# AutomationLabs-sh/AutomationLabsModelPredictiveControl.jl

Measured on AMD Instinct MI355X. Metric: MPC steps/s (batch=4096, nx=12, nu=4, N=30), higher is better.
Workload: dtype f64; 1 GPU; configs[1]: hover-linearised quadrotor nx=12 nu=4 N=30, 4096 instances per GPU, shared model, x0 amplitude classes 0.3/1.0/3.0 interleaved, cold start every step; batch_per_gpu=4096, global_batch=4096, seed=0x5eed0002, setup_ramp_steps=300, admm_max_iter=6, check_every=6, polish=1, warm_state_kept=False, parallelism=instances sharded over 1 GPU(s), 16-instance tile per workgroup

## Files before the change

automationlabsmodelpredictivecontrol.jl_amd/csrc/almpc_api.hip:

```cpp
#include "almpc_kernels.hip.h"
#include "almpc_design.hip.h"
#include "almpc_polish_gen.hip.h"
#include "almpc_fnn.hip.h"
#include "almpc_instance.hip.h"
#include "almpc_sqp.hip.h"
#include "almpc_comm.hip.h"
#include "almpc_riccati.hip.h"
#include "almpc_sdual.hip.h"
#include "almpc_host_math.h"
#include "almpc_switches.h"
#include "../../include/almpc.h"

#ifndef ALMPC_UNITY
#define ALMPC_KERNEL_INSTANCE(...) extern template __global__ __VA_ARGS__;
#include "instances/sdual_a.inc"
#include "instances/sdual_b.inc"
#include "instances/sdual_c.inc"
#include "instances/polish_gen.inc"
#include "instances/step.inc"
#include "instances/instance.inc"
#include "instances/design_a.inc"
#include "instances/design_b.inc"
#undef ALMPC_KERNEL_INSTANCE
#endif

#include <algorithm>
#include <chrono>
#include <cstdio>
#include <cstdlib>
#include <cmath>
#include <cstring>
#include <limits>
#include <string>
#include <thread>
#include <type_traits>
#include <vector>

using namespace almpc;

struct almpc_handle {
    int n = 0, m = 0, N = 0, batch = 0, nz = 0, nzs = 0, nrb = 0, ks = 0, ksf = 0, device = 0;
    uint32_t flags = 0;
    hipStream_t stream = nullptr;
    std::string err;
    bool designed = false;
    double rho = 0.1, sigma = 1e-6;
    std::vector<double> H, F, P, d;
    double *dMinvFrag = nullptr, *dVFrag = nullptr, *dHFrag = nullptr, *dFFrag = nullptr, *dG = nullptr;
    double *dD = nullptr, *dUmin = nullptr, *dUmax = nullptr, *dA = nullptr, *dB = nullptr;
    double *dXref = nullptr, *dUref = nullptr, *dFS = nullptr, *dV0S = nullptr, *dRho = nullptr;
    size_t ref_cap[3] = {0, 0, 0};
    double *wQ = nullptr, *wR = nullptr, *wS = nullptr;
    int rho_mode = 0;
    double* dRollM = nullptr;
    int roll_s = 0, roll_nb = 0;
    long xref_stride = 0, uref_stride = 0, fS_stride = 0;
    std::vector<double> hS;
    int useS = 0;
    double *dX0 = nullptr, *dXs = nullptr, *dZs = nullptr, *dYs = nullptr, *dV0 = nullptr, *dW = nullptr;
    double *dX = nullptr, *dEx = nullptr, *dU = nullptr, *dEu = nullptr;
    int32_t *dStatus = nullptr, *dIters = nullptr, *dPiters = nullptr, *dPerm = nullptr;
    uint32_t* dYflags = nullptr;
    bool state_valid = true;
    int num_cus = 256;
    Switches sw;
    int fuse_step = 1;
    double* dSglobal = nullptr;
    int32_t* dStartRows = nullptr;
    int terminal_eq = 0, has_box = 0, mc = 0, R = 0, Rs = 0, np_pairs = 0;
    double *dGhat = nullptr, *dGnorm = nullptr, *dXmin = nullptr, *dXmax = nullptr;
    int *dRowTraj = nullptr, *dRowEq = nullptr, *dRowXidx = nullptr, *dRowState = nullptr;
    double* dOvfSinv = nullptr;
    double* dVsPlain = nullptr;
    double* dPlain = nullptr;
    double* dS0Basis = nullptr;
    bool s0_basis_ok = false;
    int32_t* dOverflow = nullptr;
    int* dRowMap = nullptr;
    double *dGhatE = nullptr, *dWinvE = nullptr;
    int eq_proj = 0;
    bool ghat_inst = false;
    std::vector<double> boxmin, boxmax;
    double *lA = nullptr, *lB = nullptr, *lC = nullptr, *lE = nullptr;
    bool batched = false;
    bool ltv = false;
    double* bQ = nullptr;
    double *bA = nullptr, *bB = nullptr, *bMinv = nullptr, *bG = nullptr, *bHs = nullptr, *bFs = nullptr, *bVs = nullptr,
           *bD = nullptr, *bRho = nullptr, *bH = nullptr, *bF = nullptr;
    double *bPhi = nullptr, *bGk = nullptr, *bGam = nullptr, *bW = nullptr, *bWP = nullptr, *bP = nullptr;
    int* bFlag = nullptr;
    bool batched_alloc = false;
    bool minv_packed = false;
    struct Sqp {
        bool ready = false, started = false;
        int H = 0, L = 0, act = 0, net = 0, useR = 0, useS = 0;
        long sP = 0;
        double *W_in = nullptr, *W_h = nullptr, *b_h = nullptr, *W_out = nullptr;
        double *A = nullptr, *B = nullptr, *c = nullptr, *fval = nullptr, *ebar = nullptr, *qadd = nullptr;
        double *xref = nullptr, *uref = nullptr, *Q = nullptr, *R = nullptr, *S = nullptr;
        int* bad = nullptr;
        double* mer = nullptr;
        double *xback = nullptr, *uback = nullptr, *dxback = nullptr, *vback = nullptr;
        double mu = 0.0;
        int step_rule = 0;
        long since_start = 0;
        int structured_qp = 0;
        unsigned long long* stats = nullptr;
        int stats_cap = 0;
        int* sv = nullptr;
        double* kkt = nullptr;
        int* live_pin = nullptr;
        int hessian = 0;
        double *lam = nullptr, *Wlag = nullptr;
        int row_mult = 0;
        double* smu = nullptr;
    } sqp;
    struct Relin {
        bool ready = false;
        int H = 0, L = 0, act = 0, net = 0, useR = 0, useS = 0;
        double *W_in = nullptr, *W_h = nullptr, *b_h = nullptr, *W_out = nullptr;
        double *ulin = nullptr;
        double *Q = nullptr, *R = nullptr, *S = nullptr;
        double *gS = nullptr;
        bool have_prev = false;
        double *u0 = nullptr, *xnext = nullptr;
        double *Ascr = nullptr, *Bscr = nullptr;
        float ms_jac = 0, ms_design = 0, ms_step = 0;
        hipEvent_t ev[4] = {nullptr, nullptr, nullptr, nullptr};
    } relin;
    bool structured = false;
    struct Redo {
// ... 52 lines not shown
        hipStream_t s_in = nullptr;
        double* dX0dev[IO_DEPTH] = {nullptr, nullptr};
        hipEvent_t ev_in[IO_DEPTH] = {nullptr, nullptr};
        double* hX0[IO_DEPTH] = {nullptr, nullptr};
        double* dX0[IO_DEPTH] = {nullptr, nullptr};
        hipEvent_t ev_used[IO_DEPTH] = {nullptr, nullptr};
        bool used_pending[IO_DEPTH] = {false, false};
        int x0_slot = -1;
        double* dX0_own = nullptr;
        long x0_count = 0;
        double *hX[IO_DEPTH] = {nullptr, nullptr}, *hEx[IO_DEPTH] = {nullptr, nullptr}, *hU[IO_DEPTH] = {nullptr, nullptr},
               *hEu[IO_DEPTH] = {nullptr, nullptr}, *hU0[IO_DEPTH] = {nullptr, nullptr};
        int32_t* hInts[IO_DEPTH] = {nullptr, nullptr};
        double* dU0[IO_DEPTH] = {nullptr, nullptr};
        int32_t* dInts[IO_DEPTH] = {nullptr, nullptr};
        hipEvent_t ev_packed[IO_DEPTH] = {nullptr, nullptr};
        hipEvent_t ev_done[IO_DEPTH] = {nullptr, nullptr};
        hipEvent_t ev_big = nullptr;
        uint32_t want[IO_DEPTH] = {0, 0};
        long ticket[IO_DEPTH] = {-1, -1};
        long next_ticket = 0;
        bool big_copy_pending = false;
        int big_copy_slot = 0;
    } io;
    std::vector<hipEvent_t> ev;
    std::vector<char> ev_two;
    size_t ev_used = 0;
    int timing_stride = 1;
    size_t step_count = 0;
};

namespace {

int fail(almpc_handle* h, int code, const std::string& msg) {
    if (h) h->err = msg;
    return code;
}

#define HIP_TRY(h, call)                                                                         \
    do {                                                                                         \
        hipError_t e_ = (call);                                                                  \
        if (e_ != hipSuccess)                                                                    \
            return fail(h, ALMPC_ERR_HIP, std::string(#call) + ": " + hipGetErrorString(e_));   \
    } while (0)

template <typename T>
hipError_t dalloc(T** p, size_t count) {
    return hipMalloc(reinterpret_cast<void**>(p), count * sizeof(T) + 64);
}

int pick_ks(int nz, int nrb) {
    const int exact = (nz + 3) / 4;
    if (nrb == 8 && exact <= 30) return 30;
    if (nrb == 3 && exact <= 10) return 10;
    if (nrb == 1 && exact <= 3) return 3;
    return 4 * nrb;
}

template <int NRB, int KS>
hipError_t launch_admm_t(const AdmmParams& p, int grid, size_t lds, hipStream_t st) {
    hipLaunchKernelGGL((k_admm<NRB, KS>), dim3(grid), dim3(64 * NRB), lds, st, p);
    return hipGetLastError();
}

hipError_t launch_admm(int nrb, int ks, const AdmmParams& p, int grid, size_t lds, hipStream_t st) {
#define CASE(NRB_, KS_) if (nrb == NRB_ && ks == KS_) return launch_admm_t<NRB_, KS_>(p, grid, lds, st)
    CASE(1, 3); CASE(1, 4); CASE(2, 8); CASE(3, 10); CASE(3, 12); CASE(4, 16); CASE(5, 20); CASE(6, 24);
    CASE(7, 28); CASE(8, 30); CASE(8, 32);
#undef CASE
    return hipErrorInvalidValue;
}

void io_free(almpc_handle* h);

void io_release_x0(almpc_handle* h) {
    if (h->io.x0_slot >= 0) {
        h->dX0 = h->io.dX0_own;
        h->io.x0_slot = -1;
    }
}

void free_all(almpc_handle* h) {
    io_free(h);
    void* ptrs[] = {h->dMinvFrag, h->dVFrag, h->dHFrag, h->dFFrag, h->dG, h->dD, h->dUmin, h->dUmax, h->dA, h->dB,
                    h->dXref, h->dUref, h->dFS, h->dV0S, h->dRho, h->dRollM, h->dX0, h->dXs, h->dZs, h->dYs, h->dV0, h->dW, h->dX, h->dEx,
                    h->dU, h->dEu, h->dStatus, h->dIters, h->dPiters, h->dPerm, h->dYflags, h->dSglobal, h->dStartRows, h->dGhat, h->dGnorm, h->dXmin,
                    h->dXmax, h->dRowTraj, h->dRowEq, h->dRowXidx, h->dRowState, h->dRowMap, h->dGhatE, h->dWinvE, h->lA, h->lB, h->lC, h->lE, h->bA, h->bB, h->bMinv, h->bG, h->bHs, h->bFs,
                    h->bVs, h->bD, h->bRho, h->bH, h->bF, h->bPhi, h->bGk, h->bGam, h->bW, h->bWP, h->bP, h->bFlag, h->bQ, h->dOverflow, h->dOvfSinv, h->dVsPlain, h->dPlain, h->dS0Basis, h->wQ, h->wR, h->wS,
                    h->sqp.W_in, h->sqp.W_h, h->sqp.b_h, h->sqp.W_out, h->sqp.A, h->sqp.B, h->sqp.c, h->sqp.fval, h->sqp.ebar,
                    h->sqp.qadd, h->sqp.xref, h->sqp.uref, h->sqp.Q, h->sqp.R, h->sqp.S, h->sqp.bad, h->sqp.stats, h->sqp.mer, h->sqp.xback, h->sqp.uback, h->sqp.dxback, h->sqp.vback,
                    h->sqp.sv, h->sqp.kkt, h->sqp.lam, h->sqp.Wlag, h->sqp.smu};
    for (void* p : ptrs)
        if (p) (void)hipFree(p);
    if (h->sqp.live_pin) (void)hipHostFree(h->sqp.live_pin);
    for (void* p : {(void*)h->relin.W_in, (void*)h->relin.W_h, (void*)h->relin.b_h, (void*)h->relin.W_out, (void*)h->relin.ulin,
                    (void*)h->relin.Q, (void*)h->relin.R, (void*)h->relin.S, (void*)h->relin.gS, (void*)h->relin.u0, (void*)h->relin.xnext, (void*)h->relin.Ascr, (void*)h->relin.Bscr})
        if (p) (void)hipFree(p);
    for (auto& e : h->relin.ev)
        if (e) (void)hipEventDestroy(e);
    if (h->comm && rccl_api().ok) (void)rccl_api().CommDestroy(h->comm);
    for (void* p : {(void*)h->dComm4, (void*)h->dU0, (void*)h->dU0all, (void*)h->rQ, (void*)h->rR, (void*)h->rP, (void*)h->rKst, (void*)h->rPst, (void*)h->rGuess,
                    (void*)h->sd.rec, (void*)h->sd.base, (void*)h->sd.xmin, (void*)h->sd.xmax, (void*)h->sd.eqt, (void*)h->sd.ovf, (void*)h->sd.wsave, (void*)h->sd.sinv_glb, (void*)h->sd.ghat, (void*)h->sd.dQ, (void*)h->sd.dR, (void*)h->sd.dS, (void*)h->sd.dP, (void*)h->sd.bad, (void*)h->sd.pc, (void*)h->sd.ct,
                    (void*)h->sd.sinv_save, (void*)h->sd.start_inv, (void*)h->sd.start_ws, (void*)h->sd.scr_phi, (void*)h->sd.scr_g, (void*)h->sd.scr_rm, (void*)h->sd.scr_rp, (void*)h->sd.scr_verdict})
        if (p) (void)hipFree(p);
    if (h->ev_guess) (void)hipEventDestroy(h->ev_guess);
    if (h->ev_guess_done) (void)hipEventDestroy(h->ev_guess_done);
    if (h->redo.hUnsolved) (void)hipHostFree(h->redo.hUnsolved);
    if (h->redo.dGate) (void)hipFree(h->redo.dGate);
    for (auto& e : h->ev)
        if (e) (void)hipEventDestroy(e);
    h->ev.clear();
    if (h->stream) (void)hipStreamDestroy(h->stream);
}

int setup_state_rows(almpc_handle* h, const double* xmin, const double* xmax, bool per_instance) {
    const int n = h->n, m = h->m, N = h->N, nz = h->nz;
    h->has_box = xmin ? 1 : 0;
    std::vector<int> row_traj, row_eq, row_xidx, row_state, rowmap((size_t)N * n, -1);
    if (h->has_box)
        for (int i = 0; i < n; ++i)
            if (!(xmin[i] <= xmax[i])) return fail(h, ALMPC_ERR_INVALID, "design: xmin > xmax");
    for (int k = 0; k < N; ++k)
        for (int i = 0; i < n; ++i) {
            const bool is_eq = h->terminal_eq && k == N - 1;
            if (!(h->has_box || is_eq)) continue;
            rowmap[(size_t)k * n + i] = (int)row_traj.size();
            row_traj.push_back((k + 1) * (n + m) + i);
            row_eq.push_back(is_eq ? 1 : 0);
            row_xidx.push_back((k + 1) * n + i);
            row_state.push_back(i);
        }
    h->mc = (int)row_traj.size();
    h->R = nz + h->mc;
    h->np_pairs = (h->R + 127) / 128;
    h->Rs = 128 * h->np_pairs;
    for (void* q : {(void*)h->dGhat, (void*)h->dGnorm, (void*)h->dXmin, (void*)h->dXmax, (void*)h->dRowTraj, (void*)h->dRowEq,
                    (void*)h->dRowXidx, (void*)h->dRowState, (void*)h->dRowMap})
        if (q) (void)hipFree(q);
    h->dGhat = h->dGnorm = h->dXmin = h->dXmax = nullptr;
    h->dRowTraj = h->dRowEq = h->dRowXidx = h->dRowState = h->dRowMap = nullptr;
    h->ghat_inst = false;
    if (h->dGhatE) { (void)hipFree(h->dGhatE); h->dGhatE = nullptr; }
    if (h->dWinvE) { (void)hipFree(h->dWinvE); h->dWinvE = nullptr; }
    h->eq_proj = 0;
    if (h->mc == 0) return ALMPC_OK;
    if (h->np_pairs > 4) return fail(h, ALMPC_ERR_UNSUPPORTED, "design: state rows need n*N + m*N <= 512");
    if ((size_t)(N + 1) * (n + m) > 32 * 32) return fail(h, ALMPC_ERR_UNSUPPORTED, "design: state rows need (N+1)*(n+m) <= 1024");
    if (per_instance && n > 32) return fail(h, ALMPC_ERR_UNSUPPORTED, "design: state rows with per-instance models need n <= 32");
    const size_t copies = per_instance ? (size_t)h->batch : 1;
    HIP_TRY(h, dalloc(&h->dGhat, copies * h->R * h->Rs));
    HIP_TRY(h, dalloc(&h->dGnorm, copies * h->Rs));
    if (per_instance) HIP_TRY(h, hipMemset(h->dGhat, 0, copies * h->R * h->Rs * sizeof(double)));
    HIP_TRY(h, dalloc(&h->dXmin, (size_t)n)); HIP_TRY(h, dalloc(&h->dXmax, (size_t)n));
    HIP_TRY(h, dalloc(&h->dRowTraj, (size_t)h->Rs)); HIP_TRY(h, dalloc(&h->dRowEq, (size_t)h->Rs));
    HIP_TRY(h, dalloc(&h->dRowXidx, (size_t)h->Rs)); HIP_TRY(h, dalloc(&h->dRowState, (size_t)h->Rs));
    HIP_TRY(h, dalloc(&h->dRowMap, rowmap.size()));
    HIP_TRY(h, hipMemcpy(h->dRowMap, rowmap.data(), rowmap.size() * sizeof(int), hipMemcpyHostToDevice));
    auto up = [&](int* dst, const std::vector<int>& v, int fill) {
        std::vector<int> full((size_t)h->Rs, fill);
        for (size_t i = 0; i < v.size(); ++i) full[(size_t)nz + i] = v[i];
        return hipMemcpy(dst, full.data(), full.size() * sizeof(int), hipMemcpyHostToDevice);
    };
    HIP_TRY(h, up(h->dRowTraj, row_traj, 0)); HIP_TRY(h, up(h->dRowEq, row_eq, 0));
    HIP_TRY(h, up(h->dRowXidx, row_xidx, 0)); HIP_TRY(h, up(h->dRowState, row_state, 0));
    std::vector<double> lo(n, -1e300), hi(n, 1e300);
    if (h->has_box) { lo.assign(xmin, xmin + n); hi.assign(xmax, xmax + n); }
    HIP_TRY(h, hipMemcpy(h->dXmin, lo.data(), n * sizeof(double), hipMemcpyHostToDevice));
// ... 587 lines not shown
    bp.A = h->dA; bp.B = h->dB; bp.Vs = h->dVsPlain; bp.v0S = (h->dV0S && h->fS_stride == 0) ? h->dV0S : nullptr; bp.dvec = h->dD;
    bp.row_traj = h->dRowTraj; bp.out = h->dS0Basis;
    hipLaunchKernelGGL(k_s0_basis, dim3((unsigned)(h->n + 1)), dim3(64), (size_t)(h->N + 1) * (h->n + h->m) * sizeof(double), h->stream, bp);
    HIP_TRY(h, hipGetLastError());
    HIP_TRY(h, hipStreamSynchronize(h->stream));
    h->s0_basis_ok = true;
    return ALMPC_OK;
}

}

extern "C" {

void almpc_default_opts(almpc_opts* o) {
    if (!o) return;
    std::memset(o, 0, sizeof(*o));
    o->rho = 0.1;
    o->sigma = 1e-6;
    o->alpha = 1.6;
    o->eps_abs = 1e-3;
    o->eps_rel = 1e-3;
    o->max_iter = 25;
    o->check_every = 25;
    o->polish = 1;
    o->polish_max_iter = 0;
    o->warm_start = 0;
}

const char* almpc_last_error(const almpc_handle* h) { return h ? h->err.c_str() : "null handle"; }

int almpc_create(almpc_handle** out, int n, int m, int N, int batch, int device_id, uint32_t flags) {
    if (!out) return ALMPC_ERR_INVALID;
    *out = nullptr;
    if (n < 1 || m < 1 || N < 1 || batch < 1) return ALMPC_ERR_INVALID;
    const bool structured = (flags & ALMPC_FLAG_STRUCTURED) != 0;
    if (structured) {
        if (n > 32 || m > 16 || (long)m * N > 1024 || riccati_lds_doubles(n, m, N) * sizeof(double) > 160 * 1024) return ALMPC_ERR_UNSUPPORTED;
    } else if (n > 64 || (long)m * N > 128) return ALMPC_ERR_UNSUPPORTED;
    int count = 0;
    if (hipGetDeviceCount(&count) != hipSuccess || count < 1) return ALMPC_ERR_NO_DEVICE;
    if (device_id < 0 || device_id >= count) return ALMPC_ERR_NO_DEVICE;
    almpc_handle* h = new almpc_handle();
    h->sw = read_switches();
    h->fuse_step = h->sw.no_fused_step ? 0 : 1;
    h->n = n; h->m = m; h->N = N; h->batch = batch; h->device = device_id; h->flags = flags;
    h->structured = structured;
    h->nz = m * N;
    h->nrb = (h->nz + 15) / 16;
    h->nzs = 16 * h->nrb;
    h->ks = pick_ks(h->nz, h->nrb);
    h->ksf = (n + 3) / 4;
    auto bail = [&](int code, const std::string& msg) {
        std::fprintf(stderr, "almpc_create: %s\n", msg.c_str());
        free_all(h);
        delete h;
        return code;
    };
#define TRY(call)                                                                  \
    do {                                                                           \
        hipError_t e_ = (call);                                                    \
        if (e_ != hipSuccess) return bail(ALMPC_ERR_HIP, std::string(#call) + ": " + hipGetErrorString(e_)); \
    } while (0)
    TRY(hipSetDevice(device_id));
    TRY(hipStreamCreateWithFlags(&h->stream, hipStreamNonBlocking));
    {
        int cus = 0;
        TRY(hipDeviceGetAttribute(&cus, hipDeviceAttributeMultiprocessorCount, device_id));
        if (cus > 0) h->num_cus = cus;
    }
    const size_t fr = (size_t)h->nrb * h->ks * 64, b = (size_t)batch;
    if (structured) {
        TRY(dalloc(&h->dUmin, (size_t)m)); TRY(dalloc(&h->dUmax, (size_t)m));
        TRY(dalloc(&h->dA, (size_t)n * n)); TRY(dalloc(&h->dB, (size_t)n * m));
        TRY(dalloc(&h->dX0, b * n));
        TRY(dalloc(&h->dX, b * n * (N + 1))); TRY(dalloc(&h->dEx, b * n * (N + 1)));
        TRY(dalloc(&h->dU, b * h->nz)); TRY(dalloc(&h->dEu, b * h->nz));
        TRY(dalloc(&h->dStatus, b)); TRY(dalloc(&h->dIters, b)); TRY(dalloc(&h->dPiters, b));
        TRY(hipMemset(h->dIters, 0, b * sizeof(int32_t)));
        TRY(hipMemset(h->dX0, 0, b * n * sizeof(double)));
        *out = h;
        return ALMPC_OK;
    }
    TRY(dalloc(&h->dMinvFrag, fr)); TRY(dalloc(&h->dVFrag, (size_t)h->nrb * h->ksf * 64)); TRY(dalloc(&h->dHFrag, fr));
    TRY(dalloc(&h->dFFrag, (size_t)h->nrb * h->ksf * 64));
    TRY(dalloc(&h->dG, (size_t)h->nz * h->nzs));
    TRY(dalloc(&h->dD, (size_t)h->nzs)); TRY(dalloc(&h->dRho, (size_t)h->nzs)); TRY(dalloc(&h->dUmin, (size_t)m)); TRY(dalloc(&h->dUmax, (size_t)m));
    TRY(dalloc(&h->dA, (size_t)n * n)); TRY(dalloc(&h->dB, (size_t)n * m));
    TRY(dalloc(&h->dX0, b * n));
    TRY(dalloc(&h->dXs, b * h->nzs)); TRY(dalloc(&h->dZs, b * h->nzs)); TRY(dalloc(&h->dYs, b * h->nzs));
    TRY(dalloc(&h->dV0, b * h->nzs)); TRY(dalloc(&h->dW, b * h->nzs));
    TRY(dalloc(&h->dX, b * n * (N + 1))); TRY(dalloc(&h->dEx, b * n * (N + 1)));
    TRY(dalloc(&h->dU, b * h->nz)); TRY(dalloc(&h->dEu, b * h->nz));
    TRY(dalloc(&h->dSglobal, b * POLISH_GLB_PER_INST));
    TRY(dalloc(&h->dPerm, ((b + 15) / 16) * 16));
    TRY(hipMemset(h->dPerm, 0xFF, ((b + 15) / 16) * 16 * sizeof(int32_t)));
    TRY(dalloc(&h->dStatus, b)); TRY(dalloc(&h->dIters, b)); TRY(dalloc(&h->dPiters, b));
    TRY(dalloc(&h->dYflags, b * h->nrb));
    TRY(hipMemset(h->dXs, 0, b * h->nzs * sizeof(double)));
    TRY(hipMemset(h->dZs, 0, b * h->nzs * sizeof(double)));
    TRY(hipMemset(h->dYs, 0, b * h->nzs * sizeof(double)));
    TRY(hipMemset(h->dX0, 0, b * n * sizeof(double)));
#undef TRY
    *out = h;
    return ALMPC_OK;
}

void almpc_destroy(almpc_handle* h) {
    if (!h) return;
    (void)hipSetDevice(h->device);
    if (h->stream) (void)hipStreamSynchronize(h->stream);
    free_all(h);
    delete h;
}

int almpc_set_rho_profile(almpc_handle* h, int mode) {
    if (!h) return ALMPC_ERR_INVALID;
    if (mode != 0 && mode != 1) return fail(h, ALMPC_ERR_INVALID, "rho profile: 0 (scalar) or 1 (stiffness)");
    h->rho_mode = mode;
    h->designed = false;
    return ALMPC_OK;
}

int almpc_set_step_fusion(almpc_handle* h, int on) {
    if (!h) return ALMPC_ERR_INVALID;
    h->fuse_step = on ? 1 : 0;
    return ALMPC_OK;
}

int almpc_set_terminal_equality(almpc_handle* h, int on) {
    if (!h) return ALMPC_ERR_INVALID;
    h->terminal_eq = on ? 1 : 0;
    h->designed = false;
    return ALMPC_OK;
}

int almpc_set_state_box(almpc_handle* h, const double* xmin, const double* xmax) {
    if (!h) return ALMPC_ERR_INVALID;
    if ((xmin == nullptr) != (xmax == nullptr)) return fail(h, ALMPC_ERR_INVALID, "set_state_box: give both xmin and xmax or neither");
    if (xmin) {
        for (int i = 0; i < h->n; ++i)
            if (!(xmin[i] <= xmax[i])) return fail(h, ALMPC_ERR_INVALID, "set_state_box: xmin > xmax");
        h->boxmin.assign(xmin, xmin + h->n); h->boxmax.assign(xmax, xmax + h->n);
    } else { h->boxmin.clear(); h->boxmax.clear(); }
    h->designed = false;
    h->sqp.ready = h->sqp.started = false;
    h->relin.ready = false;
    return ALMPC_OK;
}

int almpc_set_structured_fallback(almpc_handle* h, int on) {
    if (!h) return ALMPC_ERR_INVALID;
    if (on && !riccati_shape_ok(h) && !sdual_shape_ok(h->n, h->m, h->N, false))
        return fail(h, ALMPC_ERR_UNSUPPORTED, "structured fallback: the shape is outside both stage-wise solvers");
    h->fallback = on ? 1 : 0;
    h->designed = false;
    return ALMPC_OK;
}

int almpc_set_start_from(almpc_handle* h, almpc_handle* src) {
    if (!h || !src) return ALMPC_ERR_INVALID;
    if (!h->structured) return fail(h, ALMPC_ERR_UNSUPPORTED, "set_start_from: the handle must be a structured one (ALMPC_FLAG_STRUCTURED)");
    if (!h->designed || !src->designed) return fail(h, ALMPC_ERR_NOT_DESIGNED, "set_start_from before design (of either handle)");
    if (src->n != h->n || src->m != h->m || src->batch != h->batch || src->N > h->N || src->device != h->device)
        return fail(h, ALMPC_ERR_INVALID, "set_start_from: the source must have the same n, m, batch and device and a horizon <= this handle's");
    HIP_TRY(h, hipSetDevice(h->device));
    if (!h->rGuess) HIP_TRY(h, dalloc(&h->rGuess, (size_t)h->batch * h->nz));
    if (!h->ev_guess) HIP_TRY(h, hipEventCreateWithFlags(&h->ev_guess, hipEventDisableTiming));
    HIP_TRY(h, hipEventRecord(h->ev_guess, src->stream));
    HIP_TRY(h, hipStreamWaitEvent(h->stream, h->ev_guess, 0));
    const long cnt = (long)h->batch * h->nz;
    hipLaunchKernelGGL(k_guess_from_inputs, dim3((unsigned)((cnt + 255) / 256)), dim3(256), 0, h->stream, h->batch, h->m, src->N, h->N, 0,
                       (const double*)src->dU, (const double*)h->dUref, h->uref_stride, h->rGuess);
    HIP_TRY(h, hipGetLastError());
    if (!h->ev_guess_done) HIP_TRY(h, hipEventCreateWithFlags(&h->ev_guess_done, hipEventDisableTiming));
    HIP_TRY(h, hipEventRecord(h->ev_guess_done, h->stream));
    HIP_TRY(h, hipStreamWaitEvent(src->stream, h->ev_guess_done, 0));
    h->guess_ready = true;
    return ALMPC_OK;
}

int almpc_design_shared(almpc_handle* h, const double* A, const double* B, const double* Q, const double* R,
                        const double* S, const double* P, const double* umin, const double* umax,
                        const double* xmin, const double* xmax, double rho, double sigma) {
    if (!h) return ALMPC_ERR_INVALID;
    drop_lazy_redo(h);
    if (!A || !B || !Q || !R || !umin || !umax) return fail(h, ALMPC_ERR_INVALID, "design: null matrix pointer");
    if (h->structured) {
        const int n = h->n, m = h->m, N = h->N;
        if ((xmin == nullptr) != (xmax == nullptr)) return fail(h, ALMPC_ERR_INVALID, "design: give both xmin and xmax or neither");
        for (int i = 0; i < m; ++i)
            if (!(umin[i] <= umax[i])) return fail(h, ALMPC_ERR_INVALID, "design: umin > umax");
        if (xmin)
            for (int i = 0; i < n; ++i)
                if (!(xmin[i] <= xmax[i])) return fail(h, ALMPC_ERR_INVALID, "design: xmin > xmax");
        h->designed = false;
        h->r_has_step = false; h->guess_ready = false;
        h->sqp.ready = h->sqp.started = false;
        HIP_TRY(h, hipSetDevice(h->device));
        hm::mat Am(A, A + (size_t)n * n), Bm(B, B + (size_t)n * m), Qm(Q, Q + (size_t)n * n), Rm(R, R + (size_t)m * m), Pm;
        if (P) Pm.assign(P, P + (size_t)n * n);
        else if (!hm::dare(Am, Bm, Qm, Rm, n, m, Pm)) return fail(h, ALMPC_ERR_NUMERIC, "design: DARE did not converge");
        h->P = Pm; h->H.clear(); h->F.clear(); h->d.clear();
        const bool useS = R[0] != 0.0 && S && S[0] != 0.0;
        hm::mat Rb = Rm, Sm;
        if (Rm[0] == 0.0) std::fill(Rb.begin(), Rb.end(), 0.0);
        if (useS) Sm.assign(S, S + (size_t)m * m);
        h->sd.ready = false;
        if (sdual_shape_ok(n, m, N, useS) && !h->sw.structured_primal) {
            const int rc_ = sdual_setup_shared(h, Am, Bm, Qm, Rb, useS ? &Sm : nullptr, Pm, xmin, xmax, h->terminal_eq != 0);
            if (rc_ != ALMPC_OK) return rc_;
        } else if (xmin || h->terminal_eq || useS)
            return fail(h, ALMPC_ERR_UNSUPPORTED, "structured solve: state rows / input-rate weight need the stage-wise dual solve (n + m <= 48, (N + 1)(n + m) <= 4096)");
        if (riccati_shape_ok(h)) { const int rc_ = riccati_weights(h, Qm, Rm, Pm.data()); if (rc_ != ALMPC_OK) return rc_; }
        else if (!h->sd.ready) return fail(h, ALMPC_ERR_UNSUPPORTED, "structured solve: shape outside both stage-wise solvers");
        HIP_TRY(h, hipMemcpy(h->dUmin, umin, m * sizeof(double), hipMemcpyHostToDevice));
        HIP_TRY(h, hipMemcpy(h->dUmax, umax, m * sizeof(double), hipMemcpyHostToDevice));
        HIP_TRY(h, hipMemcpy(h->dA, A, (size_t)n * n * sizeof(double), hipMemcpyHostToDevice));
        HIP_TRY(h, hipMemcpy(h->dB, B, (size_t)n * m * sizeof(double), hipMemcpyHostToDevice));
        h->batched = false; h->ltv = false; h->r_batched_P = false; h->rP_stride = 0;
        h->hS.assign((size_t)m * m, 0.0); h->useS = useS ? 1 : 0;
        if (useS) h->hS = Sm;
        h->has_box = xmin ? 1 : 0;
        h->designed = true;
        std::vector<double> xr((size_t)n * (N + 1), 0.0), ur((size_t)h->nz, 0.0);
        const int rc_ref = almpc_set_reference(h, xr.data(), ur.data(), 0);
        if (rc_ref != ALMPC_OK) h->designed = false;
        return rc_ref;
    }
    if ((xmin == nullptr) != (xmax == nullptr)) return fail(h, ALMPC_ERR_INVALID, "design: give both xmin and xmax or neither");
    if (!(rho > 0.0) || !(sigma >= 0.0)) return fail(h, ALMPC_ERR_INVALID, "design: rho must be > 0 and sigma >= 0");
    h->designed = false;
    h->sqp.ready = h->sqp.started = false;
    h->relin.ready = false;
    HIP_TRY(h, hipSetDevice(h->device));
    const int n = h->n, m = h->m, N = h->N, nz = h->nz;
    for (int i = 0; i < m; ++i)
        if (!(umin[i] <= umax[i])) return fail(h, ALMPC_ERR_INVALID, "design: umin > umax");
    hm::mat Am(A, A + (size_t)n * n), Bm(B, B + (size_t)n * m), Qm(Q, Q + (size_t)n * n), Rm(R, R + (size_t)m * m);
    hm::mat Sm = S ? hm::mat(S, S + (size_t)m * m) : hm::mat((size_t)m * m, 0.0);
    hm::mat Pm;
    if (P) Pm.assign(P, P + (size_t)n * n);
    else if (!hm::dare(Am, Bm, Qm, Rm, n, m, Pm)) return fail(h, ALMPC_ERR_NUMERIC, "design: DARE did not converge");
    h->P = Pm;
    for (int j = 0; j < m; ++j)
        for (int i = 0; i < j; ++i) {
            const double v = 0.5 * (Sm[(size_t)j * m + i] + Sm[(size_t)i * m + j]);
            Sm[(size_t)j * m + i] = Sm[(size_t)i * m + j] = v;
        }
    h->hS = Sm;
    h->useS = (Rm[0] != 0.0 && Sm[0] != 0.0) ? 1 : 0;
    h->rho = rho; h->sigma = sigma;

    { const int rc_ = setup_state_rows(h, xmin, xmax, false); if (rc_ != ALMPC_OK) return rc_; }
    std::vector<int> rowsel;
    for (int k = 0; k < N; ++k)
        for (int i = 0; i < n; ++i)
            if (h->has_box || (h->terminal_eq && k == N - 1)) rowsel.push_back(k * n + i);
    h->s0_basis_ok = false;
    if (!rowsel.empty() && !h->dVsPlain) HIP_TRY(h, dalloc(&h->dVsPlain, (size_t)n * h->nzs));
    if (h->nzs <= 64 && !h->dPlain) HIP_TRY(h, dalloc(&h->dPlain, 2 * (size_t)h->nz * h->nzs + 2 * (size_t)n * h->nzs));
    int rc = design_shared_device(h->stream, n, m, N, h->nzs, h->nrb, h->ks, h->ksf, Am, Bm, Qm, Rm, Sm, Pm, rho, sigma,
                                  h->dMinvFrag, h->dVFrag, h->dHFrag, h->dFFrag, h->dG, h->dD, h->H, h->F, h->d, h->err,
                                  rowsel, h->Rs, h->dGhat, h->dGnorm, h->rho_mode, h->dRho, rowsel.empty() ? nullptr : h->dVsPlain,
                                  h->nzs <= 64 ? h->dPlain : nullptr);
    if (rc != ALMPC_OK) return rc;
    if (h->terminal_eq && h->mc >= n && !h->sw.no_eq_projection) {
        const int ne = n, eq0 = h->R - n, Rs = h->Rs;
        std::vector<double> GE((size_t)ne * Rs), GEE((size_t)ne * ne), Y;
        HIP_TRY(h, hipMemcpy(GE.data(), h->dGhat + (size_t)eq0 * Rs, GE.size() * sizeof(double), hipMemcpyDeviceToHost));
        for (int a = 0; a < ne; ++a)
            for (int b = 0; b < ne; ++b) GEE[(size_t)b * ne + a] = GE[(size_t)a * Rs + eq0 + b];
        hm::mat Winv = hm::eye(ne);
        bool ok = hm::lu_solve(GEE, Winv, ne, ne);
        for (double v : Winv) ok = ok && std::isfinite(v);
        if (ok) {
            Y.assign((size_t)ne * Rs, 0.0);
            for (int a = 0; a < ne; ++a)
                for (int e = 0; e < ne; ++e) {
                    const double wv = Winv[(size_t)e * ne + a];
                    for (int b = 0; b < Rs; ++b) Y[(size_t)a * Rs + b] += wv * GE[(size_t)e * Rs + b];
                }
            std::vector<double> Wrow((size_t)ne * ne);
            for (int a = 0; a < ne; ++a)
                for (int e = 0; e < ne; ++e) Wrow[(size_t)a * ne + e] = Winv[(size_t)e * ne + a];
            double* dY = nullptr;
            HIP_TRY(h, dalloc(&h->dGhatE, GE.size())); HIP_TRY(h, dalloc(&h->dWinvE, Wrow.size())); HIP_TRY(h, dalloc(&dY, Y.size()));
            HIP_TRY(h, hipMemcpy(h->dGhatE, GE.data(), GE.size() * sizeof(double), hipMemcpyHostToDevice));
            HIP_TRY(h, hipMemcpy(h->dWinvE, Wrow.data(), Wrow.size() * sizeof(double), hipMemcpyHostToDevice));
            HIP_TRY(h, hipMemcpy(dY, Y.data(), Y.size() * sizeof(double), hipMemcpyHostToDevice));
            hipLaunchKernelGGL(k_ghat_project, dim3(512), dim3(256), 0, h->stream, h->R, Rs, ne, eq0, h->dGhatE, dY, h->dGhat, h->dGnorm);
            HIP_TRY(h, hipGetLastError());
            HIP_TRY(h, hipStreamSynchronize(h->stream));
            (void)hipFree(dY);
            h->eq_proj = 1;
        }
    }
    HIP_TRY(h, hipMemcpy(h->dUmin, umin, m * sizeof(double), hipMemcpyHostToDevice));
    HIP_TRY(h, hipMemcpy(h->dUmax, umax, m * sizeof(double), hipMemcpyHostToDevice));
    HIP_TRY(h, hipMemcpy(h->dA, A, (size_t)n * n * sizeof(double), hipMemcpyHostToDevice));
    HIP_TRY(h, hipMemcpy(h->dB, B, (size_t)n * m * sizeof(double), hipMemcpyHostToDevice));
    {
        int sblk = std::min(N, std::min(64 / n, ROLL_SMX / m));
        h->roll_s = 0;
        if (sblk >= 1 && n <= ROLL_NX && !h->sw.rollout_stagewise) {
            std::vector<double> M((size_t)(ROLL_SMX + ROLL_NX) * 64, 0.0);
            std::vector<hm::mat> Apow(sblk + 1), ApB(sblk);
            Apow[0] = hm::eye(n);
            for (int j = 1; j <= sblk; ++j) Apow[j] = hm::mul(Am, Apow[j - 1], n, n, n);
            for (int j = 0; j < sblk; ++j) ApB[j] = hm::mul(Apow[j], Bm, n, n, m);
            for (int j = 0; j < sblk; ++j)
                for (int i = 0; i < n; ++i) {
                    const int lane = j * n + i;
                    for (int t = 0; t <= j; ++t)
                        for (int a = 0; a < m; ++a) M[(size_t)(t * m + a) * 64 + lane] = ApB[j - t][(size_t)a * n + i];
                    for (int c = 0; c < n; ++c) M[(size_t)(ROLL_SMX + c) * 64 + lane] = Apow[j + 1][(size_t)c * n + i];
                }
            if (h->dRollM) { (void)hipFree(h->dRollM); h->dRollM = nullptr; }
            HIP_TRY(h, dalloc(&h->dRollM, M.size()));
            HIP_TRY(h, hipMemcpy(h->dRollM, M.data(), M.size() * sizeof(double), hipMemcpyHostToDevice));
            h->roll_s = sblk; h->roll_nb = (N + sblk - 1) / sblk;
        }
    }
    h->sd.ready = false;
    if (h->fallback) {
        const bool useS = h->useS != 0;
        if (sdual_shape_ok(n, m, N, useS)) {
            hm::mat Rb = Rm;
            if (Rm[0] == 0.0) std::fill(Rb.begin(), Rb.end(), 0.0);
            const int rc_ = sdual_setup_shared(h, Am, Bm, Qm, Rb, useS ? &Sm : nullptr, Pm, xmin, xmax, h->terminal_eq != 0);
            if (rc_ != ALMPC_OK && h->fallback == 1) return rc_;
        } else if (h->fallback == 1 && (h->mc > 0 || useS))
            return fail(h, ALMPC_ERR_UNSUPPORTED, "structured fallback: state rows / input-rate weight need n + m <= 48 and (N + 1)(n + m) <= 4096");
        if (riccati_shape_ok(h) && h->mc == 0 && !useS) {
            const int rc_ = riccati_weights(h, Qm, Rm, Pm.data());
            if (rc_ != ALMPC_OK) return rc_;
            h->r_batched_P = false; h->rP_stride = 0;
        }
    }
    h->designed = true;
    h->batched = false;
    h->ltv = false;
    std::vector<double> xr((size_t)n * (N + 1), 0.0), ur((size_t)nz, 0.0);
    const int rc_ref = almpc_set_reference(h, xr.data(), ur.data(), 0);
    if (rc_ref != ALMPC_OK) h->designed = false;
    return rc_ref;
// ... 401 lines not shown
        hipError_t e = upl(&dAll, ltv->A_all, b * N * n * n);
        if (e == hipSuccess) e = upl(&dBll, ltv->B_all, b * N * n * m);
        if (e == hipSuccess && ltv->c_all) e = upl(&dC, ltv->c_all, b * N * n);
        if (e == hipSuccess) e = upl(&dE, ltv->ebar, b * N * n);
        if (e == hipSuccess) e = upl(&dQa, ltv->qadd, b * nz);
        if (e == hipSuccess && !h->bQ) e = dalloc(&h->bQ, b * nz);
        if (e == hipSuccess) e = hipMemsetAsync(h->bF, 0, b * nz * n * sizeof(double), st);
        if (e == hipSuccess) {
            DesignLtvParams lp;
            lp.n = n; lp.m = m; lp.N = N; lp.nz = nz; lp.useR = useR; lp.useS = useS;
            lp.A = dAll; lp.B = dBll; lp.c = dC; lp.ebar = dE; lp.P = h->bP; lp.sP = ds.P; lp.Q = dQ; lp.R = dR; lp.S = dS;
            lp.qadd = dQa; lp.H = h->bH; lp.q = h->bQ;
            e = launch_design_ltv(h, lp, st);
        }
        if (e == hipSuccess && h->mc > 0) {
            launch_batched_factor(h, ds, rho, sigma, st, false);
            e = launch_ghat_inst(h, dAll, dBll);
        }
        if (e == hipSuccess) e = hipStreamSynchronize(st);
        for (double** q : {&h->lA, &h->lB, &h->lC, &h->lE})
            if (*q) { (void)hipFree(*q); *q = nullptr; }
        if (e == hipSuccess && h->mc > 0) {
            h->lA = dAll; h->lB = dBll; h->lC = dC; h->lE = dE;
            dAll = dBll = dC = dE = nullptr;
        }
        (void)hipFree(dAll); (void)hipFree(dBll); (void)hipFree(dC); (void)hipFree(dE); (void)hipFree(dQa);
        if (e != hipSuccess) { release(); return fail(h, ALMPC_ERR_HIP, std::string("design_ltv: ") + hipGetErrorString(e)); }
        if (h->mc == 0) launch_batched_factor(h, ds, rho, sigma, st, false);
        launch_neg_gm_batched(st, gb, nz, nzs, n, h->bG, h->bFs, h->bVs, ds.G, ds.Fs);
        BTRY(hipGetLastError());
    } else {
        BTRY(launch_batched_design(h, ds, useR, useS, dQ, dR, dS, rho, sigma, false));
        if (h->mc > 0) BTRY(launch_ghat_inst(h, nullptr, nullptr));
    }
    tr("kernels queued");
    std::vector<int> flags(b, 0);
    BTRY(hipMemcpyAsync(flags.data(), h->bFlag, b * sizeof(int), hipMemcpyDeviceToHost, st));
    h->H.assign((size_t)nz * nz, 0.0); h->F.assign((size_t)nz * n, 0.0); h->d.assign((size_t)nzs, 0.0);
    BTRY(hipMemcpyAsync(h->H.data(), h->bH, h->H.size() * sizeof(double), hipMemcpyDeviceToHost, st));
    BTRY(hipMemcpyAsync(h->F.data(), h->bF, h->F.size() * sizeof(double), hipMemcpyDeviceToHost, st));
    BTRY(hipMemcpyAsync(h->d.data(), h->bD, h->d.size() * sizeof(double), hipMemcpyDeviceToHost, st));
    BTRY(hipStreamSynchronize(st));
    tr("device done");
#undef BTRY
    release();
    tr("weights freed");
    for (size_t i = 0; i < b; ++i)
        if (flags[i] != 0)
            return fail(h, ALMPC_ERR_NUMERIC, "design_batched: instance " + std::to_string(i) +
                        (flags[i] == 1 ? ": condensed Hessian has a non-positive diagonal" : ": Cholesky pivot not positive"));
    HIP_TRY(h, hipMemcpy(h->dUmin, umin, m * sizeof(double), hipMemcpyHostToDevice));
    HIP_TRY(h, hipMemcpy(h->dUmax, umax, m * sizeof(double), hipMemcpyHostToDevice));
    h->sd.ready = false;
    if (h->fallback && !ltv) {
        h->r_batched_P = true; h->rP_stride = p_inst ? (long)n * n : 0;
        if (sdual_shape_ok(n, m, N, useS != 0)) {
            const int rc_ = sdual_setup_batched(h, Qm, Rm, useS ? &Sm : nullptr, P == nullptr && !useS,
                                                h->boxmin.empty() ? nullptr : h->boxmin.data(), h->boxmax.empty() ? nullptr : h->boxmax.data(), h->terminal_eq != 0);
            if (rc_ != ALMPC_OK && h->fallback == 1) return rc_;
        } else if (h->fallback == 1 && (h->mc > 0 || useS))
            return fail(h, ALMPC_ERR_UNSUPPORTED, "structured fallback: state rows / input-rate weight need n + m <= 48 and (N + 1)(n + m) <= 4096");
        if (riccati_shape_ok(h) && h->mc == 0 && !useS) {
            const int rc_ = riccati_weights(h, Qm, Rm, nullptr);
            if (rc_ != ALMPC_OK) return rc_;
        }
    }
    h->designed = true;
    h->batched = true;
    h->ltv = false;
    if (!ltv) {
        std::vector<double> xr((size_t)n * (N + 1), 0.0), ur((size_t)nz, 0.0);
        const int rc = almpc_set_reference(h, xr.data(), ur.data(), 0);
        if (rc != ALMPC_OK) h->designed = false;
        tr("flags + set_reference");
        return rc;
    }
    {
        const int rc = almpc_set_reference(h, ltv->xbar, ltv->ubar, 1);
        if (rc != ALMPC_OK) { h->designed = false; return rc; }
    }
    h->designed = false;
    hipLaunchKernelGGL(k_fs_scale, dim3(256), dim3(256), 0, h->stream, h->batch, nz, nzs, h->bQ, (long)nz, h->bD, h->dFS);
    hipLaunchKernelGGL(k_neg_gm, dim3(1, (unsigned)h->batch), dim3(256), 0, h->stream, nz, nzs, 1, nz, h->bG, h->dFS, h->dV0S,
                       (long)nz * nzs, (long)nz);
    HIP_TRY(h, hipGetLastError());
    HIP_TRY(h, hipStreamSynchronize(h->stream));
    h->ltv = true;
    h->designed = true;
    return ALMPC_OK;
}
}

namespace {
int relin_setup_structured(almpc_handle* h, int H, int L, int net, int activation, const double* W_in, const double* W_h, const double* b_h,
                           const double* W_out, const double* xref, const double* uref, const double* Q, const double* R, const double* S,
                           const double* P, const double* umin, const double* umax) {
    const int n = h->n, m = h->m, N = h->N, nz = h->nz;
    const size_t b = (size_t)h->batch, nin = (size_t)n + m;
    if (fnn_wave_scratch_doubles(n, m, H, L, net) * sizeof(double) > 160 * 1024)
        return fail(h, ALMPC_ERR_UNSUPPORTED, "relin_fnn_setup: the network's forward-mode Jacobian must fit the 160 KB of LDS");
    for (int i = 0; i < m; ++i)
        if (!(umin[i] <= umax[i])) return fail(h, ALMPC_ERR_INVALID, "relin_fnn_setup: umin > umax");
    h->designed = false;
    h->sqp.ready = h->sqp.started = false;
    h->relin.ready = false;
    HIP_TRY(h, hipSetDevice(h->device));
    HIP_TRY(h, hipStreamSynchronize(h->stream));
    auto sym = [](const double* M, int k) {
        hm::mat o((size_t)k * k, 0.0);
        if (M)
            for (int j = 0; j < k; ++j)
                for (int i = 0; i < k; ++i) o[(size_t)j * k + i] = 0.5 * (M[(size_t)j * k + i] + M[(size_t)i * k + j]);
        return o;
    };
    const hm::mat Qm = sym(Q, n), Rm = sym(R, m), Sm = sym(S, m), Pm = sym(P, n);
    const bool useS = Rm[0] != 0.0 && S && Sm[0] != 0.0;
    if (!sdual_shape_ok(n, m, N, useS))
        return fail(h, ALMPC_ERR_UNSUPPORTED, "relin_fnn_setup (structured): n (+ m with an input-rate weight) <= 48, m <= 16 and (N + 1)(n + m) <= 4096");
    almpc_handle::Relin& q = h->relin;
    for (void* p_ : {(void*)q.W_in, (void*)q.W_h, (void*)q.b_h, (void*)q.W_out, (void*)q.ulin, (void*)q.Q, (void*)q.R, (void*)q.S, (void*)q.gS})
        if (p_) (void)hipFree(p_);
    q.W_in = q.W_h = q.b_h = q.W_out = q.ulin = q.Q = q.R = q.S = q.gS = nullptr;
    auto up = [&](double** d, const double* src, size_t cnt) -> hipError_t {
        hipError_t e = dalloc(d, cnt ? cnt : 1);
        if (e == hipSuccess && src && cnt) e = hipMemcpy(*d, src, cnt * sizeof(double), hipMemcpyHostToDevice);
        return e;
    };
    std::vector<double> xr((size_t)n * (N + 1), 0.0), ur((size_t)nz, 0.0);
    if (xref) xr.assign(xref, xref + xr.size());
    if (uref) ur.assign(uref, uref + ur.size());
    std::vector<double> ul(b * m);
    for (size_t i = 0; i < b; ++i)
        for (int a = 0; a < m; ++a) ul[i * m + a] = ur[a];
    HIP_TRY(h, up(&q.W_in, W_in, (size_t)H * nin)); HIP_TRY(h, up(&q.W_h, W_h, net_wh_doubles(net, H, L))); HIP_TRY(h, up(&q.b_h, b_h, (size_t)L * H));
    HIP_TRY(h, up(&q.W_out, W_out, net_wout_doubles(net, n, H, L))); HIP_TRY(h, up(&q.ulin, ul.data(), ul.size()));
    if (!h->bA) HIP_TRY(h, dalloc(&h->bA, b * n * n));
    if (!h->bB) HIP_TRY(h, dalloc(&h->bB, b * n * m));
    if (!h->bP) HIP_TRY(h, dalloc(&h->bP, b * n * n));
    HIP_TRY(h, hipMemset(h->bA, 0, b * n * n * sizeof(double)));
    HIP_TRY(h, hipMemset(h->bB, 0, b * n * m * sizeof(double)));
    HIP_TRY(h, hipMemcpy(h->bP, Pm.data(), Pm.size() * sizeof(double), hipMemcpyHostToDevice));
    h->batched = true; h->ltv = false; h->r_batched_P = true; h->rP_stride = 0;
    h->sd.ready = false;
    {
        const int rc_ = sdual_setup_batched(h, Qm, Rm, useS ? &Sm : nullptr, false, h->boxmin.empty() ? nullptr : h->boxmin.data(),
                                            h->boxmax.empty() ? nullptr : h->boxmax.data(), h->terminal_eq != 0);
        if (rc_ != ALMPC_OK) return rc_;
    }
    if (riccati_shape_ok(h)) { const int rc_ = riccati_weights(h, Qm, Rm, nullptr); if (rc_ != ALMPC_OK) return rc_; }
    HIP_TRY(h, hipMemcpy(h->dUmin, umin, m * sizeof(double), hipMemcpyHostToDevice));
    HIP_TRY(h, hipMemcpy(h->dUmax, umax, m * sizeof(double), hipMemcpyHostToDevice));
    h->P = Pm; h->H.clear(); h->F.clear(); h->d.clear();
    h->hS = Sm; h->useS = useS ? 1 : 0;
    h->has_box = h->boxmin.empty() ? 0 : 1;
    for (auto& e : q.ev)
        if (!e) HIP_TRY(h, hipEventCreate(&e));
    q.H = H; q.L = L; q.act = activation; q.net = net; q.have_prev = false; q.useR = Rm[0] != 0.0; q.useS = useS;
    if (!q.u0) HIP_TRY(h, dalloc(&q.u0, b * m));
    if (!q.xnext) HIP_TRY(h, dalloc(&q.xnext, b * n));
    h->r_has_step = false;
    h->designed = true;
    const int rc_ref = almpc_set_reference(h, xr.data(), ur.data(), 0);
    if (rc_ref != ALMPC_OK) { h->designed = false; return rc_ref; }
    q.ready = true;
    return ALMPC_OK;
}


enum class Guess { Admm, FromIterate, ShiftInputs };
struct StepMode {
    Guess guess = Guess::Admm;
    bool fold_flag = false;
    RowMultOut rows;
};

struct StepTimer {
    hipEvent_t* ev = nullptr;
    hipStream_t st = nullptr;
    bool started = false;
    hipError_t open(almpc_handle* h) {
        st = h->stream;
        if (!(h->flags & ALMPC_FLAG_TIMING) || (h->step_count++ % (size_t)h->timing_stride) != 0) return hipSuccess;
        if (h->ev.size() < 4 * (h->ev_used + 1)) {
            const size_t old = h->ev.size();
            h->ev.resize(old + 4 * 64, nullptr);
            for (size_t i = old; i < h->ev.size(); ++i) {
                const hipError_t e = hipEventCreate(&h->ev[i]);
                if (e != hipSuccess) return e;
            }
        }
        ev = &h->ev[4 * h->ev_used];
        if (h->ev_two.size() < h->ev_used + 1) h->ev_two.resize(h->ev_used + 64, 0);
        return hipSuccess;
    }
    hipError_t start() {
        if (!ev || started) return hipSuccess;
        started = true;
        return hipEventRecord(ev[0], st);
    }
    hipError_t mark(int i) const { return ev ? hipEventRecord(ev[i], st) : hipSuccess; }
    hipError_t close(almpc_handle* h) const {
        if (!ev) return hipSuccess;
        if (started) {
            const hipError_t e = hipEventRecord(ev[3], st);
            if (e != hipSuccess) return e;
        }
        h->ev_two[h->ev_used] = started ? 0 : 1;
        h->ev_used += 1;
        return hipSuccess;
    }
};

struct Step {
    almpc_handle* h;
    almpc_opts o;
    StepMode mode;
    bool keep_state, lazy_redo;
    StepTimer t;
    RollGeom roll;
    RolloutParams rp;
};

AdmmInstParams admm_inst_params(const almpc_handle* h, const almpc_opts& o, bool shared) {
    AdmmInstParams ip;
    ip.nz = h->nz; ip.n = h->n; ip.m = h->m; ip.batch = h->batch; ip.nzs = h->nzs;
    if (shared) {
        const size_t mm = (size_t)h->nz * h->nzs, fv = (size_t)h->n * h->nzs;
        ip.Minv = h->dPlain; ip.Hs = h->dPlain + mm; ip.Fs = h->dPlain + 2 * mm; ip.Vs = h->dPlain + 2 * mm + fv;
        ip.dvec = h->dD; ip.rhovec = h->dRho;
        ip.mat_stride = 0; ip.fv_stride = 0; ip.vec_stride = 0; ip.fs_stride = h->fS_stride;
    } else {
        ip.Minv = h->bMinv; ip.Hs = h->bHs; ip.Fs = h->bFs; ip.Vs = h->bVs; ip.dvec = h->bD; ip.rhovec = h->bRho;
        ip.mat_stride = (long)h->nz * h->nzs; ip.fv_stride = (long)h->n * h->nzs; ip.vec_stride = h->nzs; ip.fs_stride = h->nz;
    }
    ip.fS = h->dFS; ip.v0S = h->dV0S; ip.umin = h->dUmin; ip.umax = h->dUmax;
    ip.uref = h->dUref; ip.uref_stride = h->uref_stride; ip.xref = h->dXref; ip.xref_stride = h->xref_stride; ip.x0 = h->dX0;
    ip.xs = h->dXs; ip.zs = h->dZs; ip.ys = h->dYs; ip.v0 = h->dV0; ip.status = h->dStatus; ip.iters = h->dIters;
    ip.piters = h->dPiters; ip.perm = h->dPerm;
    ip.sigma = o.sigma; ip.alpha = o.alpha; ip.eps_abs = o.eps_abs; ip.eps_rel = o.eps_rel;
    ip.max_iter = o.max_iter; ip.check_every = o.check_every; ip.warm = o.warm_start ? 1 : 0;
    return ip;
}

AdmmParams admm_params(const almpc_handle* h, const almpc_opts& o, bool keep_state) {
    AdmmParams ap;
    ap.nz = h->nz; ap.n = h->n; ap.m = h->m; ap.batch = h->batch; ap.nzs = h->nzs;
    ap.MinvFrag = h->dMinvFrag; ap.VFrag = h->dVFrag; ap.v0S = h->dV0S; ap.v0S_stride = h->fS_stride; ap.HFrag = h->dHFrag; ap.FFrag = h->dFFrag; ap.ksf = h->ksf;
    ap.dvec = h->dD; ap.rhovec = h->dRho; ap.umin = h->dUmin; ap.umax = h->dUmax;
    ap.uref = h->dUref; ap.uref_stride = h->uref_stride; ap.xref = h->dXref; ap.xref_stride = h->xref_stride;
    ap.fS = h->dFS; ap.fS_stride = h->fS_stride; ap.x0 = h->dX0;
    ap.xs = h->dXs; ap.zs = h->dZs; ap.ys = h->dYs; ap.v0 = h->dV0; ap.status = h->dStatus; ap.iters = h->dIters;
    ap.piters = h->dPiters;
    ap.perm = h->dPerm;
    ap.rho = o.rho; ap.sigma = o.sigma; ap.alpha = o.alpha; ap.eps_abs = o.eps_abs; ap.eps_rel = o.eps_rel;
    ap.max_iter = o.max_iter; ap.check_every = o.check_every; ap.warm = o.warm_start ? 1 : 0;
    ap.keep_state = keep_state ? 1 : 0; ap.yflags = h->dYflags;
    return ap;
}

size_t admm_lds_bytes(const almpc_handle* h) {
    return ((size_t)2 * h->nzs * TILE + (size_t)h->nrb * 8 * TILE + (size_t)4 * h->ksf * TILE) * sizeof(double);
}

RolloutParams rollout_params(const almpc_handle* h) {
    RolloutParams rp;
    rp.n = h->n; rp.m = h->m; rp.N = h->N; rp.batch = h->batch; rp.nzs = h->nzs; rp.A = h->batched ? h->bA : h->dA; rp.B = h->batched ? h->bB : h->dB;
    rp.dvec = h->dD; rp.w = h->dZs; rp.x0 = h->dX0; rp.xref = h->dXref; rp.xref_stride = h->xref_stride;
    rp.uref = h->dUref; rp.uref_stride = h->uref_stride; rp.umin = h->dUmin; rp.umax = h->dUmax; rp.x = h->dX; rp.ex = h->dEx; rp.u = h->dU; rp.eu = h->dEu;
    return rp;
}

struct PolishLayout {
    PolishShared SL;
    bool fused = false;
    int fuse_rollout = 0;
    int per_wave = 0;
    int wave_const_off = -1;
    int sg_shared_off = -1;
    size_t g_lds = 0;
    size_t l_glds = 0, l_step = 0;
};

PolishLayout polish_layout(const almpc_handle* h, const RollGeom& roll) {
    PolishLayout L;
    const bool blocked = !h->batched && h->roll_s > 0;
    L.fused = roll.fits || blocked;
    L.fuse_rollout = L.fused ? (h->ltv ? 2 : (blocked ? 3 : 1)) : 0;
    int per_wave = POLISH_LDS_MIN_PER_WAVE;
    if (L.fused && !blocked && (h->N + 1) * (h->n + h->m) > per_wave) per_wave = (h->N + 1) * (h->n + h->m);
    per_wave = (per_wave + 1) & ~1;
    if (h->batched) {
        L.wave_const_off = per_wave;
        per_wave += (h->nzs + h->n * (h->n + h->m) + 1) & ~1;
    }
    L.per_wave = per_wave;
    L.SL = polish_shared_layout(h->n, h->m, h->N, h->nz, h->nzs, L.fuse_rollout);
    L.g_lds = (size_t)h->nz * ((h->nz + 1) & ~1);
    L.l_glds = (L.g_lds + L.SL.total + (size_t)POLISH_WAVES_GLDS * per_wave + 2) * sizeof(double);
    const size_t slot = (size_t)POLISH_SG_SHARED_CAP * 64 * sizeof(double);
    if (L.l_glds + slot <= 160 * 1024 && !h->batched && !h->sw.polish_sg_global) {
        L.sg_shared_off = (int)(L.SL.total + (size_t)POLISH_WAVES_GLDS * per_wave + 2);
        L.l_glds += slot;
    }
    L.l_step = L.l_glds - L.g_lds * sizeof(double);
    if (admm_lds_bytes(h) > L.l_step) L.l_step = admm_lds_bytes(h);
    L.l_step += L.g_lds * sizeof(double);
    return L;
}

PolishParams polish_params(const Step& s, const PolishLayout& L) {
    const almpc_handle* h = s.h;
    PolishParams pp;
    pp.nz = h->nz; pp.m = h->m; pp.batch = h->batch; pp.nzs = h->nzs;
    pp.G = h->batched ? h->bG : h->dG; pp.dvec = h->batched ? h->bD : h->dD;
    pp.G_stride = h->batched ? (long)h->nz * h->nzs : 0; pp.d_stride = h->batched ? (long)h->nzs : 0;
    pp.A_stride = h->batched ? (long)h->n * h->n : 0; pp.B_stride = h->batched ? (long)h->n * h->m : 0;
    pp.wave_const_off = L.wave_const_off; pp.sg_off = 0; pp.g_off = 0; pp.sg_shared_off = L.sg_shared_off;
    pp.umin = h->dUmin; pp.umax = h->dUmax; pp.uref = h->dUref; pp.uref_stride = h->uref_stride;
    pp.zs = h->dZs; pp.ys = h->dYs; pp.v0 = h->dV0; pp.w = h->dW; pp.status = h->dStatus; pp.piters = h->dPiters;
    pp.yflags = s.keep_state ? nullptr : h->dYflags; pp.yflag_words = h->nrb;
    pp.sglobal = h->dSglobal; pp.perm = h->dPerm; pp.ntiles = (h->batch + 15) / 16;
    pp.max_iter = s.o.polish_max_iter > 0 ? s.o.polish_max_iter : 2 * h->nz + 50;
    pp.dflag = s.mode.fold_flag ? h->bFlag : nullptr;
    if (s.lazy_redo) { pp.unsolved = h->redo.dUnsolved; pp.redo_gate = h->redo.dGate; pp.step_serial = h->redo.step_serial; }
    pp.fuse_rollout = L.fuse_rollout; pp.roll_g = s.roll.g; pp.roll_cpl = s.roll.cpl; pp.roll = s.rp;
    pp.rollM = h->dRollM; pp.roll_s = h->roll_s; pp.roll_nb = h->roll_nb;
    pp.lds_per_wave = L.per_wave;
    return pp;
}

// ... 471 lines not shown
    for (auto& e : q.ev)
        if (!e) HIP_TRY(h, hipEventCreate(&e));
    q.H = H; q.L = L; q.act = activation; q.net = net; q.have_prev = false;
    if (!q.u0) HIP_TRY(h, dalloc(&q.u0, b * m));
    if (!q.xnext) HIP_TRY(h, dalloc(&q.xnext, b * n));
    h->P = Pm; h->hS = Sm; h->useS = q.useS;
    h->rho = rho; h->sigma = sigma;
    { const int rc_ = setup_state_rows(h, h->boxmin.empty() ? nullptr : h->boxmin.data(), h->boxmax.empty() ? nullptr : h->boxmax.data(), true);
      if (rc_ != ALMPC_OK) return rc_; }
    h->batched = true; h->ltv = false;
    h->state_valid = true;
    h->sd.ready = false;
    if (h->fallback) {
        h->r_batched_P = true; h->rP_stride = 0;
        if (sdual_shape_ok(n, m, N, q.useS != 0)) {
            const int rc_ = sdual_setup_batched(h, Qm, Rm, q.useS ? &Sm : nullptr, false,
                                                h->boxmin.empty() ? nullptr : h->boxmin.data(), h->boxmax.empty() ? nullptr : h->boxmax.data(), h->terminal_eq != 0);
            if (rc_ != ALMPC_OK && h->fallback == 1) return rc_;
            if (rc_ == ALMPC_OK) { const int rb_ = sdual_update_base(h, ur.data(), 1); if (rb_ != ALMPC_OK) return rb_; }
        } else if (h->fallback == 1 && (h->mc > 0 || q.useS))
            return fail(h, ALMPC_ERR_UNSUPPORTED, "structured fallback: state rows / input-rate weight need n + m <= 48 and (N + 1)(n + m) <= 4096");
        if (riccati_shape_ok(h) && h->mc == 0 && !q.useS) {
            const int rc_ = riccati_weights(h, Qm, Rm, nullptr);
            if (rc_ != ALMPC_OK) return rc_;
        }
    }
    q.ready = true;
    return ALMPC_OK;
}
int almpc_relin_fnn_setup(almpc_handle* h, int H, int L, int activation, const double* W_in, const double* W_h, const double* b_h,
                          const double* W_out, const double* xref, const double* uref, const double* Q, const double* R,
                          const double* S, const double* P, const double* umin, const double* umax, double rho, double sigma) {
    return relin_net_setup(h, false, H, L, activation, W_in, W_h, b_h, W_out, xref, uref, Q, R, S, P, umin, umax, rho, sigma);
}
int almpc_relin_densenet_setup(almpc_handle* h, int H, int L, int activation, const double* W_in, const double* W_h, const double* b_h,
                               const double* W_out, const double* xref, const double* uref, const double* Q, const double* R,
                               const double* S, const double* P, const double* umin, const double* umax, double rho, double sigma) {
    return relin_net_setup(h, true, H, L, activation, W_in, W_h, b_h, W_out, xref, uref, Q, R, S, P, umin, umax, rho, sigma);
}

int almpc_relin_fnn_step_async(almpc_handle* h, const almpc_opts* opts) {
    if (!h) return ALMPC_ERR_INVALID;
    almpc_handle::Relin& q = h->relin;
    if (!q.ready) return fail(h, ALMPC_ERR_NOT_DESIGNED, "relin_fnn_step before relin_fnn_setup");
    HIP_TRY(h, hipSetDevice(h->device));
    const int n = h->n, m = h->m, nz = h->nz, nzs = h->nzs;
    hipStream_t st = h->stream;
    const bool timing = (h->flags & ALMPC_FLAG_TIMING) != 0;
    if (timing) HIP_TRY(h, hipEventRecord(q.ev[0], st));
    FnnParams fp;
    fp.n = n; fp.m = m; fp.H = q.H; fp.L = q.L; fp.act = q.act; fp.batch = h->batch;
    fp.W_in = q.W_in; fp.W_h = q.W_h; fp.b_h = q.b_h; fp.W_out = q.W_out;
    fp.x = h->dX0; fp.u = q.ulin; fp.ppi = 1; fp.xs_group = n; fp.us_group = m;
    fp.A = h->bA; fp.B = h->bB; fp.f = nullptr;
    if (h->structured) {
        HIP_TRY(h, launch_fnn_jacobian(h->sw, fp, q.net, h->num_cus, st));
        if (timing) HIP_TRY(h, hipEventRecord(q.ev[1], st));
        HIP_TRY(h, launch_sgains(h, 0));
        if (timing) HIP_TRY(h, hipEventRecord(q.ev[2], st));
        h->designed = true;
        almpc_opts o2;
        almpc_default_opts(&o2);
        if (opts) o2 = *opts;
        if (!q.have_prev) o2.warm_start = 0;
        const int rc = almpc_calculate_async(h, &o2);
        if (rc != ALMPC_OK) { h->designed = false; return rc; }
        q.have_prev = true;
        if (timing) HIP_TRY(h, hipEventRecord(q.ev[3], st));
        return ALMPC_OK;
    }
    const bool fuse_jac = design_fuses_fnn(h, q.H, q.L, q.net);
    if (!fuse_jac) HIP_TRY(h, launch_fnn_jacobian(h->sw, fp, q.net, h->num_cus, st));
    if (timing) HIP_TRY(h, hipEventRecord(q.ev[1], st));
    const bool warm = opts && opts->warm_start && q.have_prev && (!opts || opts->polish);
    const DesignStrides ds = batched_strides(h, false);
    {
        const hipError_t e_ = launch_batched_design(h, ds, q.useR, q.useS, q.Q, q.R, q.S, h->rho, h->sigma, warm, fuse_jac ? &fp : nullptr);
        if (e_ != hipSuccess) return fail(h, ALMPC_ERR_HIP, std::string("relin design: ") + hipGetErrorString(e_));
    }
    if (h->mc > 0) HIP_TRY(h, launch_ghat_inst(h, nullptr, nullptr));
    if (q.useS) {
        hipLaunchKernelGGL(k_fs_scale, dim3(256), dim3(256), 0, st, h->batch, nz, nzs, q.gS, 0L, h->bD, h->dFS);
        hipLaunchKernelGGL(k_neg_gm, dim3(1, (unsigned)h->batch), dim3(256), 0, st, nz, nzs, 1, nz, h->bG, h->dFS, h->dV0S,
                           (long)nz * nzs, (long)nz);
        HIP_TRY(h, hipGetLastError());
    }
    if (timing) HIP_TRY(h, hipEventRecord(q.ev[2], st));
    h->designed = true;
    almpc_opts o2;
    almpc_default_opts(&o2);
    if (opts) o2 = *opts;
    o2.warm_start = 0;
    StepMode mode;
    mode.guess = warm ? Guess::ShiftInputs : Guess::Admm;
    mode.fold_flag = h->mc == 0 && o2.polish != 0;
    const int rc = calculate_checked(h, &o2, mode);
    if (rc != ALMPC_OK) { h->designed = false; return rc; }
    q.have_prev = true;
    if (!mode.fold_flag) {
        hipLaunchKernelGGL(k_flag_to_status, dim3((h->batch + 255) / 256), dim3(256), 0, st, h->batch, h->bFlag, h->dStatus);
        HIP_TRY(h, hipGetLastError());
    }
    if (timing) HIP_TRY(h, hipEventRecord(q.ev[3], st));
    return ALMPC_OK;
}

int almpc_relin_fnn_step(almpc_handle* h, const almpc_opts* opts) {
    const int rc = almpc_relin_fnn_step_async(h, opts);
    if (rc != ALMPC_OK) return rc;
    return almpc_synchronize(h);
}

int almpc_relin_fnn_advance(almpc_handle* h) {
    if (!h) return ALMPC_ERR_INVALID;
    almpc_handle::Relin& q = h->relin;
    if (!q.ready || !q.have_prev) return fail(h, ALMPC_ERR_NOT_DESIGNED, "relin_fnn_advance needs a solved almpc_relin_fnn_step");
    HIP_TRY(h, hipSetDevice(h->device));
    { const int rc_ = enqueue_gated_redo(h); if (rc_ != ALMPC_OK) return rc_; }
    const int n = h->n, m = h->m;
    hipStream_t st = h->stream;
    const size_t cnt = (size_t)h->batch * m;
    hipLaunchKernelGGL(k_pack_first_input, dim3((unsigned)((cnt + 255) / 256)), dim3(256), 0, st, h->batch, m, h->N, h->dU, q.u0);
    FnnParams fp;
    fp.n = n; fp.m = m; fp.H = q.H; fp.L = q.L; fp.act = q.act; fp.batch = h->batch;
    fp.W_in = q.W_in; fp.W_h = q.W_h; fp.b_h = q.b_h; fp.W_out = q.W_out;
    fp.x = h->dX0; fp.u = q.u0; fp.ppi = 1; fp.xs_group = n; fp.us_group = m;
    if (!q.Ascr) { HIP_TRY(h, dalloc(&q.Ascr, (size_t)h->batch * n * n)); HIP_TRY(h, dalloc(&q.Bscr, (size_t)h->batch * n * m)); }
    fp.A = q.Ascr; fp.B = q.Bscr; fp.f = q.xnext;
    HIP_TRY(h, launch_fnn_jacobian(h->sw, fp, q.net, h->num_cus, st));
    if (h->io.x0_slot >= 0) {
        HIP_TRY(h, hipEventRecord(h->io.ev_used[h->io.x0_slot], st));
        h->io.used_pending[h->io.x0_slot] = true;
    }
    io_release_x0(h);
    HIP_TRY(h, hipMemcpyAsync(h->dX0, q.xnext, (size_t)h->batch * n * sizeof(double), hipMemcpyDeviceToDevice, st));
    return ALMPC_OK;
}

int almpc_relin_fnn_timing(almpc_handle* h, float* ms_jacobian, float* ms_design, float* ms_step) {
    if (!h) return ALMPC_ERR_INVALID;
    if (!(h->flags & ALMPC_FLAG_TIMING) || !h->relin.ready) return fail(h, ALMPC_ERR_INVALID, "relin_fnn_timing: needs ALMPC_FLAG_TIMING and a step");
    HIP_TRY(h, hipSetDevice(h->device));
    HIP_TRY(h, hipEventSynchronize(h->relin.ev[3]));
    float a = 0, d = 0, s2 = 0;
    HIP_TRY(h, hipEventElapsedTime(&a, h->relin.ev[0], h->relin.ev[1]));
    HIP_TRY(h, hipEventElapsedTime(&d, h->relin.ev[1], h->relin.ev[2]));
    HIP_TRY(h, hipEventElapsedTime(&s2, h->relin.ev[2], h->relin.ev[3]));
    if (ms_jacobian) *ms_jacobian = a;
    if (ms_design) *ms_design = d;
    if (ms_step) *ms_step = s2;
    return ALMPC_OK;
}

static int sqp_net_setup(almpc_handle* h, bool dense, int H, int L, int activation, const double* W_in, const double* W_h,
                         const double* b_h, const double* W_out, const double* xref, const double* uref, const double* Q,
                         const double* R, const double* S, const double* P, int P_per_instance, const double* umin, const double* umax,
                         double rho, double sigma) {
    if (!h) return ALMPC_ERR_INVALID;
    drop_lazy_redo(h);
    if (H < 1 || L < 0 || !W_in || !W_out || (L > 0 && (!W_h || !b_h)) || !Q || !R || !P || !umin || !umax)
        return fail(h, ALMPC_ERR_INVALID, "sqp_fnn_setup: null pointer or bad network shape (P must be given)");
    int net = NET_FNN;
    if (!setup_net(dense, activation, &net, &activation))
        return fail(h, ALMPC_ERR_UNSUPPORTED, dense ? "sqp_densenet_setup: activation must be 0..4"
                                                    : "sqp_fnn_setup: activation must be ALMPC_NET_CODE(kind 0..2, activation 0..4)");
    if (!(rho > 0.0) || !(sigma >= 0.0)) return fail(h, ALMPC_ERR_INVALID, "sqp_fnn_setup: rho must be > 0 and sigma >= 0");
    const int n = h->n, m = h->m, N = h->N, nz = h->nz, nzs = h->nzs;
// ... 348 lines not shown
            return fail(h, ALMPC_ERR_UNSUPPORTED, "sqp row multipliers: the condensed QP route only (the stage-wise route of "
                                                  "almpc_sqp_fnn_set_structured / ALMPC_FLAG_STRUCTURED does not hand them out)");
        { const int rc_ = sqp_rows_buffer(h); if (rc_ != ALMPC_OK) return rc_; }
        rows.mu = q.smu; rows.done = sv ? sv->done : nullptr; rows.mer = q.step_rule ? q.mer : nullptr;
    }
    bool all_done = false;
    DesignLtvParams lp;
    lp.n = n; lp.m = m; lp.N = N; lp.nz = nz; lp.useR = q.useR; lp.useS = q.useS;
    lp.A = q.A; lp.B = q.B; lp.c = q.c; lp.ebar = q.ebar; lp.P = h->bP; lp.sP = q.sP; lp.Q = q.Q; lp.R = q.R; lp.S = q.S;
    lp.qadd = q.qadd; lp.H = h->bH; lp.q = h->bQ;
    const bool exact = q.hessian == 1;
    FnnHessParams hp;
    SqpExactParams xp;
    size_t hess_lds = 0, exact_lds = 0;
    if (exact) {
        { const int rc_ = sqp_exact_check(h); if (rc_ != ALMPC_OK) return rc_; }
        if (!q.lam) { HIP_TRY(h, dalloc(&q.lam, b * N * (size_t)n)); HIP_TRY(h, dalloc(&q.Wlag, b * N * (size_t)(n + m) * (n + m))); }
        if (!sv) {
            kp.n = n; kp.m = m; kp.N = N; kp.nz = nz; kp.useS = q.useS;
            kp.xref = q.xref; kp.uref = q.uref; kp.Q = q.Q; kp.R = q.R; kp.S = q.S; kp.P = h->bP; kp.sP = q.sP;
            kp.umin = h->dUmin; kp.umax = h->dUmax; kp.xbar = h->dXref; kp.ubar = h->dUref; kp.fval = q.fval; kp.A = q.A; kp.B = q.B;
            kp.tol = 0.0; kp.it = 0; kp.done = nullptr; kp.iters = nullptr; kp.kkt = nullptr; kp.live = nullptr;
            if (step_lds > 64 * 1024) HIP_TRY(h, ensure_dyn_lds(reinterpret_cast<const void*>(k_sqp_kkt), (size_t)(step_lds)));
        }
        kp.lam = q.lam;
        hp.n = n; hp.m = m; hp.H = q.H; hp.L = q.L; hp.act = q.act; hp.N = N; hp.batch = h->batch;
        hp.W_in = q.W_in; hp.W_h = q.W_h; hp.b_h = q.b_h; hp.W_out = q.W_out; hp.xbar = h->dXref; hp.ubar = h->dUref; hp.lam = q.lam;
        hp.done = sv ? sv->done : nullptr; hp.W = q.Wlag;
        xp.n = n; xp.m = m; xp.N = N; xp.nz = nz; xp.A = q.A; xp.B = q.B; xp.c = q.c; xp.W = q.Wlag; xp.ubar = h->dUref;
        xp.umin = h->dUmin; xp.umax = h->dUmax; xp.done = sv ? sv->done : nullptr; xp.H = h->bH; xp.q = h->bQ;
        hess_lds = 4 * fnn_hess_wave_doubles(n, m, q.H, q.L, q.net) * sizeof(double);
        exact_lds = sqp_exact_lds_doubles(n, m, nz) * sizeof(double);
    }
    if (rows.mu) {
        kp.mu = q.smu; kp.term_eq = h->terminal_eq ? 1 : 0;
        if (h->has_box) { kp.xmin = h->dXmin; kp.xmax = h->dXmax; }
    }
    const bool ltv_scales = !exact && ltv_reg_path(h) && nz <= 128 && !q.structured_qp && !h->sw.dbg_split_scale;
    if (ltv_scales) { lp.sc_d = h->bD; lp.sc_Hs = h->bHs; lp.sc_fS = h->dFS; lp.sc_flag = h->bFlag; lp.nzs = nzs; }
    const bool prep_in_design = ltv_scales && !h->sw.dbg_split_prepare;
    if (prep_in_design) { lp.prep_on = 1; lp.prep = sp; }
    for (int it = 0; it < iters; ++it) {
        if (sv && it >= 2) {
            HIP_TRY(h, hipEventSynchronize(sv->ev[(it - 2) & 3]));
            if (sv->live_pin[(it - 2) & 3] == 0) { all_done = true; break; }
        }
        HIP_TRY(h, launch_fnn_jacobian(h->sw, fp, q.net, h->num_cus, st));
        if (sv) HIP_TRY(h, kkt_test(it));
        if (exact) {
            if (!sv) hipLaunchKernelGGL(k_sqp_kkt, dim3((unsigned)b), dim3(256), step_lds, st, kp);
            void (*hk)(FnnHessParams) = with_net(q.net, [](auto k) { return k_fnn_lag_hessian<k>; });
            hipLaunchKernelGGL(hk, dim3((unsigned)((b * N + 3) / 4)), dim3(256), hess_lds, st, hp);
            HIP_TRY(h, hipGetLastError());
        }
        if (!prep_in_design) hipLaunchKernelGGL(k_sqp_prepare, dim3((unsigned)b), dim3(256), 0, st, sp);
        if (!ltv_scales) HIP_TRY(h, hipMemsetAsync(h->bFlag, 0, b * sizeof(int), st));
        if (q.structured_qp) {
            h->designed = true;
            if (h->mc == 0 && !q.useS && h->rKst)
                HIP_TRY(h, launch_riccati(h, 3, h->dUref, opts ? opts->polish_max_iter : 0));
            else if (h->sd.ready) {
                HIP_TRY(h, launch_sgains(h, 0));
                HIP_TRY(h, launch_sdual(h, 0, h->dUref, opts ? opts->polish_max_iter : 0, false, h->nz > 48 ? 1 : 0));
            } else
                return fail(h, ALMPC_ERR_UNSUPPORTED, "sqp_fnn_iterate: no stage-wise QP solver for this design");
            q.since_start += 1;
            sp.stats = q.stats + 2 * it;
            hipLaunchKernelGGL(k_sqp_step, dim3((unsigned)b), dim3(256), step_lds, st, sp);
            HIP_TRY(h, hipGetLastError());
            continue;
        }
        HIP_TRY(h, launch_design_ltv(h, lp, st));
        if (exact) {
            hipLaunchKernelGGL(k_sqp_exact_qp, dim3((unsigned)b), dim3(256), exact_lds, st, xp);
            HIP_TRY(h, hipGetLastError());
        }
        StepMode mode;
        mode.guess = (!h->sw.sqp_admm_always && q.since_start > 0) ? Guess::FromIterate : Guess::Admm;
        mode.rows = rows;
        const bool v0_in_inverse = ltv_scales && design_inverse_makes_v(h->sw, nz);
        launch_batched_factor(h, ds, h->rho, h->sigma, st, mode.guess != Guess::Admm, ltv_scales, false, v0_in_inverse ? h->dFS : nullptr, h->dV0S);
        if (h->mc > 0) HIP_TRY(h, launch_ghat_inst(h, q.A, q.B));
        if (!ltv_scales) hipLaunchKernelGGL(k_fs_scale, dim3(256), dim3(256), 0, st, h->batch, nz, nzs, h->bQ, (long)nz, h->bD, h->dFS);
        if (!v0_in_inverse) hipLaunchKernelGGL(k_neg_gm, dim3(1, (unsigned)b), dim3(256), 0, st, nz, nzs, 1, nz, h->bG, h->dFS, h->dV0S, (long)nz * nzs, (long)nz);
        HIP_TRY(h, hipGetLastError());
        h->designed = true;
        const int rc = calculate_checked(h, opts, mode);
        if (rc != ALMPC_OK) return rc;
        if (h->fallback) {
            const bool primal_only = h->mc == 0 && !q.useS && h->rKst && !h->sw.sqp_redo_dual_first;
            if (h->sd.ready && !primal_only) { HIP_TRY(h, launch_sgains(h, 2)); HIP_TRY(h, launch_sdual(h, 2, nullptr, 0, true, 0, {}, rows)); }
            if (h->mc == 0 && !q.useS && h->rKst) HIP_TRY(h, launch_riccati(h, 2, nullptr, 0));
        }
        q.since_start += 1;
        sp.stats = q.stats + 2 * it;
        hipLaunchKernelGGL(k_sqp_step, dim3((unsigned)b), dim3(256), step_lds, st, sp);
        HIP_TRY(h, hipGetLastError());
    }
    if (sv && !all_done) {
        HIP_TRY(h, launch_fnn_jacobian(h->sw, fp, q.net, h->num_cus, st));
        HIP_TRY(h, kkt_test(iters));
    }
    if (sv) return almpc_synchronize(h);
    std::vector<unsigned long long> stats((size_t)2 * iters);
    std::vector<int> bad(b);
    HIP_TRY(h, hipMemcpyAsync(stats.data(), q.stats, stats.size() * sizeof(unsigned long long), hipMemcpyDeviceToHost, st));
    HIP_TRY(h, hipMemcpyAsync(bad.data(), q.bad, b * sizeof(int), hipMemcpyDeviceToHost, st));
    { const int rc = almpc_synchronize(h); if (rc != ALMPC_OK) return rc; }
    for (int it = 0; it < iters; ++it) {
        double a, c2;
        std::memcpy(&a, &stats[2 * it], 8); std::memcpy(&c2, &stats[2 * it + 1], 8);
        if (step_inf) step_inf[it] = a;
        if (defect_inf) defect_inf[it] = c2;
    }
    for (size_t i = 0; i < b; ++i)
        if (bad[i])
            return fail(h, ALMPC_ERR_NUMERIC, "sqp_fnn_iterate: instance " + std::to_string(i) +
                        ": an iteration was skipped (condensed Hessian not positive definite to working precision, a non-finite QP "
                        "solution, or -- with state rows -- an infeasible QP); its iterate is the last good one, the other instances are unaffected");
    return ALMPC_OK;
}

int almpc_sqp_fnn_set_structured(almpc_handle* h, int on) {
    if (!h) return ALMPC_ERR_INVALID;
    if (on && !riccati_shape_ok(h) && !sdual_shape_ok(h->n, h->m, h->N, false))
        return fail(h, ALMPC_ERR_UNSUPPORTED, "sqp_fnn_set_structured: the shape is outside both stage-wise QP solvers");
    h->sqp.structured_qp = on ? 1 : 0;
    h->designed = false;
    h->sqp.ready = h->sqp.started = false;
    return ALMPC_OK;
}

int almpc_sqp_fnn_set_step_rule(almpc_handle* h, int rule) {
    if (!h) return ALMPC_ERR_INVALID;
    if (rule != 0 && rule != 1) return fail(h, ALMPC_ERR_INVALID, "sqp_fnn_set_step_rule: 0 (fixed step) or 1 (merit-function safeguard)");
    h->sqp.step_rule = rule;
    return ALMPC_OK;
}

int almpc_sqp_fnn_set_row_multipliers(almpc_handle* h, int on) {
    if (!h) return ALMPC_ERR_INVALID;
    h->sqp.row_mult = on ? 1 : 0;
    return ALMPC_OK;
}

int almpc_sqp_fnn_state_multipliers(almpc_handle* h, double* mu) {
    if (!h || !mu) return ALMPC_ERR_INVALID;
    if (!h->sqp.ready) return fail(h, ALMPC_ERR_NOT_DESIGNED, "sqp_fnn_state_multipliers before sqp_fnn_setup");
    const size_t cnt = (size_t)h->batch * h->N * h->n;
    if (!h->sqp.smu) {
        std::fill(mu, mu + cnt, 0.0);
        return ALMPC_OK;
    }
    HIP_TRY(h, hipSetDevice(h->device));
    HIP_TRY(h, hipStreamSynchronize(h->stream));
    HIP_TRY(h, hipMemcpy(mu, h->sqp.smu, cnt * sizeof(double), hipMemcpyDeviceToHost));
    return ALMPC_OK;
}

int almpc_sqp_fnn_skipped(almpc_handle* h, int32_t* skipped) {
    if (!h || !skipped) return ALMPC_ERR_INVALID;
    if (!h->sqp.ready) return fail(h, ALMPC_ERR_NOT_DESIGNED, "sqp_fnn_skipped before sqp_fnn_setup");
    HIP_TRY(h, hipSetDevice(h->device));
    HIP_TRY(h, hipStreamSynchronize(h->stream));
    HIP_TRY(h, hipMemcpy(skipped, h->sqp.bad, (size_t)h->batch * sizeof(int), hipMemcpyDeviceToHost));
    return ALMPC_OK;
}

int almpc_get_design_instance(almpc_handle* h, int instance, double* H, double* F, double* d) {
    if (!h) return ALMPC_ERR_INVALID;
    if (!h->designed || !h->batched) return fail(h, ALMPC_ERR_NOT_DESIGNED, "get_design_instance needs almpc_design_batched");
    if (instance < 0 || instance >= h->batch) return fail(h, ALMPC_ERR_INVALID, "get_design_instance: instance out of range");
    HIP_TRY(h, hipSetDevice(h->device));
    HIP_TRY(h, hipStreamSynchronize(h->stream));
    const size_t nz = h->nz, n = h->n, i = (size_t)instance;
    if (H) HIP_TRY(h, hipMemcpy(H, h->bH + i * nz * nz, nz * nz * sizeof(double), hipMemcpyDeviceToHost));
    if (F) HIP_TRY(h, hipMemcpy(F, h->bF + i * nz * n, nz * n * sizeof(double), hipMemcpyDeviceToHost));
    if (d) HIP_TRY(h, hipMemcpy(d, h->bD + i * h->nzs, nz * sizeof(double), hipMemcpyDeviceToHost));
    return ALMPC_OK;
}

int almpc_set_reference(almpc_handle* h, const double* xref, const double* uref, int per_instance) {
    if (!h) return ALMPC_ERR_INVALID;
    if (!h->designed) return fail(h, ALMPC_ERR_NOT_DESIGNED, "set_reference before design");
    if (h->ltv) return fail(h, ALMPC_ERR_INVALID, "set_reference: the references of an LTV design are arguments of almpc_design_ltv");
    if (h->relin.ready)
        return fail(h, ALMPC_ERR_INVALID, "set_reference: the references of the re-linearisation pipeline are arguments of almpc_relin_fnn_setup");
    if (!xref || !uref) return fail(h, ALMPC_ERR_INVALID, "set_reference: null pointer");
    HIP_TRY(h, hipSetDevice(h->device));
    const int n = h->n, m = h->m, N = h->N, nz = h->nz;
    const size_t cnt = per_instance ? (size_t)h->batch : 1;
    const size_t xs = (size_t)n * (N + 1), us = (size_t)nz;
    HIP_TRY(h, hipStreamSynchronize(h->stream));
    if (h->structured) {
        h->designed = false;
        if (h->dXref) { (void)hipFree(h->dXref); h->dXref = nullptr; }
        if (h->dUref) { (void)hipFree(h->dUref); h->dUref = nullptr; }
        h->ref_cap[0] = h->ref_cap[1] = h->ref_cap[2] = 0;
        HIP_TRY(h, dalloc(&h->dXref, cnt * xs));
        HIP_TRY(h, dalloc(&h->dUref, cnt * us));
        HIP_TRY(h, hipMemcpy(h->dXref, xref, cnt * xs * sizeof(double), hipMemcpyHostToDevice));
        HIP_TRY(h, hipMemcpy(h->dUref, uref, cnt * us * sizeof(double), hipMemcpyHostToDevice));
        h->xref_stride = per_instance ? (long)xs : 0;
        h->uref_stride = per_instance ? (long)us : 0;
        { const int rc_ = sdual_update_base(h, uref, cnt); if (rc_ != ALMPC_OK) return rc_; }
        h->designed = true;
        return ALMPC_OK;
    }
    h->sqp.ready = h->sqp.started = false;
    h->relin.ready = false;
    h->designed = false;
    const size_t fcnt = h->batched ? (size_t)h->batch : cnt;
    if (!(h->dXref && h->dUref && h->dFS && h->dV0S && h->ref_cap[0] == cnt * xs && h->ref_cap[1] == cnt * us && h->ref_cap[2] == fcnt * us)) {
        if (h->dXref) { (void)hipFree(h->dXref); h->dXref = nullptr; }
        if (h->dUref) { (void)hipFree(h->dUref); h->dUref = nullptr; }
        if (h->dFS) { (void)hipFree(h->dFS); h->dFS = nullptr; }
        if (h->dV0S) { (void)hipFree(h->dV0S); h->dV0S = nullptr; }
        h->ref_cap[0] = h->ref_cap[1] = h->ref_cap[2] = 0;
        HIP_TRY(h, dalloc(&h->dXref, cnt * xs));
        HIP_TRY(h, dalloc(&h->dUref, cnt * us));
        HIP_TRY(h, dalloc(&h->dFS, fcnt * us));
        HIP_TRY(h, dalloc(&h->dV0S, fcnt * us));
        h->ref_cap[0] = cnt * xs; h->ref_cap[1] = cnt * us; h->ref_cap[2] = fcnt * us;
    }
    HIP_TRY(h, hipMemcpy(h->dXref, xref, cnt * xs * sizeof(double), hipMemcpyHostToDevice));
    HIP_TRY(h, hipMemcpy(h->dUref, uref, cnt * us * sizeof(double), hipMemcpyHostToDevice));
    std::vector<double> fS(cnt * us, 0.0);
    if (h->useS) {
        for (size_t c = 0; c < cnt; ++c) {
            const double* ur = uref + c * us;
            double* f = fS.data() + c * us;
            for (int i = 0; i + 1 < N; ++i)
                for (int a = 0; a < m; ++a) {
                    double sd = 0.0;
                    for (int b2 = 0; b2 < m; ++b2) sd += h->hS[(size_t)b2 * m + a] * (ur[i * m + b2] - ur[(i + 1) * m + b2]);
                    f[i * m + a] += 2.0 * sd;
                    f[(i + 1) * m + a] -= 2.0 * sd;
                }
            if (!h->batched)
                for (int r = 0; r < nz; ++r) f[r] *= h->d[r];
        }
    }
    if (h->batched && !h->useS) {
        HIP_TRY(h, hipMemsetAsync(h->dFS, 0, fcnt * us * sizeof(double), h->stream));
        HIP_TRY(h, hipMemsetAsync(h->dV0S, 0, fcnt * us * sizeof(double), h->stream));
        HIP_TRY(h, hipStreamSynchronize(h->stream));
    } else if (h->batched) {
        double* dGs = nullptr;
        HIP_TRY(h, dalloc(&dGs, cnt * us));
        hipError_t e = hipMemcpy(dGs, fS.data(), cnt * us * sizeof(double), hipMemcpyHostToDevice);
        if (e == hipSuccess) {
            hipLaunchKernelGGL(k_fs_scale, dim3(256), dim3(256), 0, h->stream, h->batch, nz, h->nzs, dGs, per_instance ? (long)us : 0L,
                               h->bD, h->dFS);
            hipLaunchKernelGGL(k_neg_gm, dim3(1, (unsigned)h->batch), dim3(256), 0, h->stream, nz, h->nzs, 1, (int)us, h->bG, h->dFS,
                               h->dV0S, (long)nz * h->nzs, (long)us);
            e = hipGetLastError();
            if (e == hipSuccess) e = hipStreamSynchronize(h->stream);
        }
        (void)hipFree(dGs);
        if (e != hipSuccess) return fail(h, ALMPC_ERR_HIP, std::string("set_reference (batched): ") + hipGetErrorString(e));
    } else {
    HIP_TRY(h, hipMemcpy(h->dFS, fS.data(), cnt * us * sizeof(double), hipMemcpyHostToDevice));
    {
        const size_t blocks = (cnt * us + 255) / 256;
        hipLaunchKernelGGL(k_neg_gm, dim3((unsigned)(blocks < 1024 ? blocks : 1024)), dim3(256), 0, h->stream, nz, h->nzs,
                           (int)cnt, (int)us, h->dG, h->dFS, h->dV0S, 0L, 0L);
        HIP_TRY(h, hipGetLastError());
        HIP_TRY(h, hipStreamSynchronize(h->stream));
    }
    }
    h->xref_stride = per_instance ? (long)xs : 0;
    h->uref_stride = per_instance ? (long)us : 0;
    h->fS_stride = (per_instance || h->batched) ? (long)us : 0;
    { const int rc_ = sdual_update_base(h, uref, cnt); if (rc_ != ALMPC_OK) return rc_; }
    { const int rc_ = build_s0_basis(h); if (rc_ != ALMPC_OK) return rc_; }
    h->designed = true;
    return ALMPC_OK;
}

int almpc_update_initialization(almpc_handle* h, const double* x0) {
    if (!h || !x0) return h ? fail(h, ALMPC_ERR_INVALID, "update_initialization: null x0") : ALMPC_ERR_INVALID;
    HIP_TRY(h, hipSetDevice(h->device));
    io_release_x0(h);
    HIP_TRY(h, hipMemcpyAsync(h->dX0, x0, (size_t)h->batch * h->n * sizeof(double), hipMemcpyHostToDevice, h->stream));
    HIP_TRY(h, hipStreamSynchronize(h->stream));
    return ALMPC_OK;
}

int almpc_update_initialization_device(almpc_handle* h, const double* d_x0) {
    if (!h || !d_x0) return h ? fail(h, ALMPC_ERR_INVALID, "update_initialization_device: null x0") : ALMPC_ERR_INVALID;
    HIP_TRY(h, hipSetDevice(h->device));
    io_release_x0(h);
    HIP_TRY(h, hipMemcpyAsync(h->dX0, d_x0, (size_t)h->batch * h->n * sizeof(double), hipMemcpyDeviceToDevice, h->stream));
    return ALMPC_OK;
}

int almpc_calculate_async(almpc_handle* h, const almpc_opts* user) { return calculate_checked(h, user, StepMode()); }

int almpc_synchronize(almpc_handle* h) {
    if (!h) return ALMPC_ERR_INVALID;
    HIP_TRY(h, hipSetDevice(h->device));
    return wait_and_settle(h);
}

int almpc_calculate(almpc_handle* h, const almpc_opts* opts) {
    int rc = almpc_calculate_async(h, opts);
    if (rc != ALMPC_OK) return rc;
    return almpc_synchronize(h);
}

int almpc_get_results(almpc_handle* h, double* x, double* e_x, double* u, double* e_u, int32_t* status,
                      int32_t* iters, int32_t* polish_iters) {
    if (!h) return ALMPC_ERR_INVALID;
    if (!h->designed) return fail(h, ALMPC_ERR_NOT_DESIGNED, "get_results before design");
    HIP_TRY(h, hipSetDevice(h->device));
    { const int rc_ = wait_and_settle(h, true); if (rc_ != ALMPC_OK) return rc_; }
    const size_t b = (size_t)h->batch, xs = (size_t)h->n * (h->N + 1), us = (size_t)h->nz;
    if (x) HIP_TRY(h, hipMemcpy(x, h->dX, b * xs * sizeof(double), hipMemcpyDeviceToHost));
    if (e_x) HIP_TRY(h, hipMemcpy(e_x, h->dEx, b * xs * sizeof(double), hipMemcpyDeviceToHost));
    if (u) HIP_TRY(h, hipMemcpy(u, h->dU, b * us * sizeof(double), hipMemcpyDeviceToHost));
    if (e_u) HIP_TRY(h, hipMemcpy(e_u, h->dEu, b * us * sizeof(double), hipMemcpyDeviceToHost));
    if (status) HIP_TRY(h, hipMemcpy(status, h->dStatus, b * sizeof(int32_t), hipMemcpyDeviceToHost));
    if (iters) HIP_TRY(h, hipMemcpy(iters, h->dIters, b * sizeof(int32_t), hipMemcpyDeviceToHost));
    if (polish_iters) HIP_TRY(h, hipMemcpy(polish_iters, h->dPiters, b * sizeof(int32_t), hipMemcpyDeviceToHost));
    return ALMPC_OK;
}

int almpc_get_design(almpc_handle* h, double* H, double* F, double* P, double* d) {
    if (!h) return ALMPC_ERR_INVALID;
    if (!h->designed) return fail(h, ALMPC_ERR_NOT_DESIGNED, "get_design before design");
    if (H) std::memcpy(H, h->H.data(), h->H.size() * sizeof(double));
    if (F) std::memcpy(F, h->F.data(), h->F.size() * sizeof(double));
    if (P) std::memcpy(P, h->P.data(), h->P.size() * sizeof(double));
    if (d && h->d.size() >= (size_t)h->nz) std::memcpy(d, h->d.data(), (size_t)h->nz * sizeof(double));
    return ALMPC_OK;
}

int almpc_device_results(almpc_handle* h, const double** d_x, const double** d_e_x, const double** d_u,
                         const double** d_e_u) {
    if (!h) return ALMPC_ERR_INVALID;
    if (d_x) *d_x = h->dX;
    if (d_e_x) *d_e_x = h->dEx;
    if (d_u) *d_u = h->dU;
    if (d_e_u) *d_e_u = h->dEu;
    return ALMPC_OK;
}

int almpc_timing_set_stride(almpc_handle* h, int every) {
    if (!h || every < 1) return ALMPC_ERR_INVALID;
    h->timing_stride = every;
    h->step_count = 0;
    return ALMPC_OK;
// ... 275 lines not shown
```

automationlabsmodelpredictivecontrol.jl_amd/csrc/almpc_design.hip.h:

```cpp
#pragma once
#include "almpc_kernels.hip.h"
#include "almpc_switches.h"

#include <string>
#include <vector>

namespace almpc {

struct DesignStrides {
    long A = 0, B = 0, P = 0, Phi = 0, Gk = 0, Gam = 0, WP = 0, H = 0, F = 0, d = 0, Hs = 0, Fs = 0, G = 0, Minv = 0, rho = 0,
         flag = 0;
    int h_symmetric = 0;
};

inline __global__ __launch_bounds__(256) void k_design_blocks(int n, int m, int N, const double* A, const double* B,
                                                       double* Phi, double* Gk, DesignStrides st) {
    extern __shared__ __attribute__((aligned(16))) double smem[];
    A += blockIdx.y * st.A; B += blockIdx.y * st.B; Phi += blockIdx.y * st.Phi; Gk += blockIdx.y * st.Gk;
    double* As = smem;
    double* Bs = As + n * n;
    double* cur = Bs + n * m;
    double* nxt = cur + n * n;
    for (int t = threadIdx.x; t < n * n; t += blockDim.x) {
        As[t] = A[t];
// ... 655 lines not shown
inline void launch_design_inverse(const Switches& sw, dim3 grid, size_t lds, hipStream_t st, int nz, int nzs, const double* Hs, double cshift, const double* dshift,
                                  double* Out, int* flag, long sHs, long sShift, long sOut, long sFlag,
                                  const double* rho_G = nullptr, long sRhoG = 0, int rho_mode = 0, double rho = 0.0, double* rho_out = nullptr,
                                  const double* vM = nullptr, double* vOut = nullptr, long sV = 0, int vcols = 0,
                                  double* Out2 = nullptr, long sOut2 = 0, double cshift2 = 0.0, int vld = 0, int packed_out = 0) {
    if (vld == 0) vld = nzs;
    if (nz <= 64 && !sw.inv_tile) {
        const int b = (int)grid.y;
        const dim3 g2((unsigned)(((Out2 ? 2 * b : b) + 3) / 4));
#define INV_WAVE(NC_) hipLaunchKernelGGL((k_design_inverse_wave<NC_>), g2, dim3(256), 0, st, nz, nzs, b, Hs, cshift, dshift, Out, flag, sHs, sShift, sOut, sFlag, rho_G, sRhoG, rho_mode, rho, rho_out, vM, vOut, sV, vcols, Out2, sOut2, cshift2, vld)
        if (nz <= 16) INV_WAVE(16); else if (nz <= 32) INV_WAVE(32); else if (nz <= 48) INV_WAVE(48); else INV_WAVE(64);
#undef INV_WAVE
    } else if (nz <= 64) hipLaunchKernelGGL((k_design_inverse_t<2, 8>), grid, dim3(DESIGN_INVERSE_THREADS), lds, st, nz, nzs, Hs, cshift, dshift, Out, flag, sHs, sShift, sOut, sFlag);
    else if (!sw.inv_tile) {
        const long cw = sw.inv_columns_per_wave.value_or(grid.y <= 256 ? 16 : 32);
#define INV_C32(CW_, H_) hipLaunchKernelGGL((k_design_inverse_c32<CW_, H_>), grid, dim3(64 * (128 / CW_)), 0, st, nz, nzs, Hs, cshift, dshift, Out, flag, sHs, sShift, sOut, sFlag, vM, vOut, sV, vcols, vld, packed_out)
        if (grid.y <= 256) { if (cw == 8) INV_C32(8, true); else if (cw == 16) INV_C32(16, true); else INV_C32(32, true); }
        else { if (cw == 8) INV_C32(8, false); else if (cw == 16) INV_C32(16, false); else INV_C32(32, false); }
#undef INV_C32
    }
    else hipLaunchKernelGGL((k_design_inverse_t<4, 16>), grid, dim3(DESIGN_INVERSE_THREADS), lds, st, nz, nzs, Hs, cshift, dshift, Out, flag, sHs, sShift, sOut, sFlag);
}

inline __global__ __launch_bounds__(512) void k_design_inverse_chol(int nz, int nzs, const double* Hs, double cshift, const double* dshift,
                                                        double* Out, int* flag, long sHs, long sShift, long sOut, long sFlag) {
    extern __shared__ __attribute__((aligned(16))) double smem[];
    Hs += blockIdx.y * sHs; Out += blockIdx.y * sOut; flag += blockIdx.y * sFlag;
    if (dshift) dshift += blockIdx.y * sShift;
    const int ld = nz + 1;
    double* L = smem;
    double* xo = L + (size_t)nz * ld;
    int* badp = reinterpret_cast<int*>(xo + nz);
    if (threadIdx.x == 0) *badp = 0;
    for (int t = threadIdx.x; t < nz * nz; t += blockDim.x) {
        const int i = t % nz, j = t / nz;
        L[j * ld + i] = Hs[(size_t)j * nzs + i] + (i == j ? cshift + (dshift ? dshift[i] : 0.0) : 0.0);
    }
    __syncthreads();
    for (int j = 0; j < nz; ++j) {
        const double piv = L[j * ld + j];
        if (!(piv > 0.0)) { if (threadIdx.x == 0) *badp = 1; }
        const double ljj = sqrt(piv > 0.0 ? piv : 1.0);
        __syncthreads();
        for (int i = j + threadIdx.x; i < nz; i += blockDim.x) L[j * ld + i] = (i == j) ? ljj : L[j * ld + i] / ljj;
        __syncthreads();
        const int rem = nz - j - 1;
        for (int t = threadIdx.x; t < rem * rem; t += blockDim.x) {
            const int i = j + 1 + t % rem, k = j + 1 + t / rem;
            if (i >= k) L[k * ld + i] -= L[j * ld + i] * L[j * ld + k];
        }
        __syncthreads();
    }
    for (int j = nz - 1; j >= 0; --j) {
        const double ajj = 1.0 / L[j * ld + j];
        for (int i = j + 1 + threadIdx.x; i < nz; i += blockDim.x) {
            double s = 0.0;
            for (int k = j + 1; k <= i; ++k) s += L[k * ld + i] * L[j * ld + k];
            xo[i] = -s * ajj;
        }
        __syncthreads();
        for (int i = j + threadIdx.x; i < nz; i += blockDim.x) L[j * ld + i] = (i == j) ? ajj : xo[i];
        __syncthreads();
    }
    for (int t = threadIdx.x; t < nz * nz; t += blockDim.x) {
        const int i = t % nz, j = t / nz;
        if (i < j) continue;
        double s = 0.0;
        for (int k = i; k < nz; ++k) s += L[i * ld + k] * L[j * ld + k];
        Out[(size_t)j * nzs + i] = s;
        Out[(size_t)i * nzs + j] = s;
    }
    __syncthreads();
    if (threadIdx.x == 0 && *badp) atomicExch(flag, 2);
}

inline __global__ __launch_bounds__(256) void k_design_rho(int nz, int nzs, int mode, double rho, const double* G, double* rhovec,
                                                    long sG, long sRho) {
    G += blockIdx.y * sG; rhovec += blockIdx.y * sRho;
    for (int t = threadIdx.x; t < nzs; t += blockDim.x)
        rhovec[t] = (t < nz) ? (mode == 1 ? rho / G[(size_t)t * nzs + t] : rho) : 1.0;
}

inline __global__ __launch_bounds__(256) void k_pack_frags(const double* M, int rows, int cols, int ld, int nrb, int ks,
                                                    double* frag) {
    const int total = nrb * ks * 64;
    for (int t = blockIdx.x * blockDim.x + threadIdx.x; t < total; t += gridDim.x * blockDim.x) {
        const int l = t & 63, s = (t >> 6) % ks, rb = (t >> 6) / ks;
        const int r = rb * 16 + (l & 15), c = 4 * s + (l >> 4);
        frag[t] = (r < rows && c < cols) ? M[(size_t)c * ld + r] : 0.0;
    }
}

inline __global__ __launch_bounds__(256) void k_neg_gm(int nz, int nzs, int ncols, int ld, const double* G, const double* M, double* Out,
                                                long sG, long sM) {
    G += blockIdx.y * sG; M += blockIdx.y * sM; Out += blockIdx.y * sM;
    for (long t = (long)blockIdx.x * blockDim.x + threadIdx.x; t < (long)ncols * nz; t += (long)gridDim.x * blockDim.x) {
        const int c = (int)(t / nz), r = (int)(t % nz);
        const double* mcol = M + (size_t)c * ld;
        double a0 = 0.0, a1 = 0.0, a2 = 0.0, a3 = 0.0;
        int j = 0;
        for (; j + 8 <= nz; j += 8) {
            double g[8], mv[8];
#pragma unroll
            for (int u = 0; u < 8; ++u) { g[u] = G[(size_t)(j + u) * nzs + r]; mv[u] = mcol[j + u]; }
            a0 += g[0] * mv[0] + g[4] * mv[4];
            a1 += g[1] * mv[1] + g[5] * mv[5];
            a2 += g[2] * mv[2] + g[6] * mv[6];
            a3 += g[3] * mv[3] + g[7] * mv[7];
        }
        for (; j < nz; ++j) a0 += G[(size_t)j * nzs + r] * mcol[j];
        Out[(size_t)c * ld + r] = -((a0 + a1) + (a2 + a3));
    }
}

template <int NC>
__global__ __launch_bounds__(128) void k_neg_gm_cols(int nz, int nzs, int ncols, int ld, const double* G, const double* M, double* Out,
                                                     long sG, long sM) {
    extern __shared__ __attribute__((aligned(16))) double smem[];
    G += blockIdx.y * sG; M += blockIdx.y * sM; Out += blockIdx.y * sM;
    for (int t = threadIdx.x; t < ncols * nz; t += blockDim.x) smem[t] = M[(size_t)(t / nz) * ld + t % nz];
    __syncthreads();
    const int r = threadIdx.x < nz ? threadIdx.x : nz - 1;
    double a[NC][4];
#pragma unroll
    for (int c = 0; c < NC; ++c) { a[c][0] = 0.0; a[c][1] = 0.0; a[c][2] = 0.0; a[c][3] = 0.0; }
    int j = 0;
    for (; j + 8 <= nz; j += 8) {
        double g[8];
#pragma unroll
        for (int u = 0; u < 8; ++u) g[u] = G[(size_t)(j + u) * nzs + r];
#pragma unroll
        for (int c = 0; c < NC; ++c)
            if (c < ncols) {
                const double* mv = smem + c * nz + j;
                a[c][0] += g[0] * mv[0] + g[4] * mv[4];
                a[c][1] += g[1] * mv[1] + g[5] * mv[5];
                a[c][2] += g[2] * mv[2] + g[6] * mv[6];
                a[c][3] += g[3] * mv[3] + g[7] * mv[7];
            }
    }
    for (; j < nz; ++j) {
        const double gv = G[(size_t)j * nzs + r];
#pragma unroll
        for (int c = 0; c < NC; ++c)
            if (c < ncols) a[c][0] += gv * smem[c * nz + j];
    }
    if (threadIdx.x < nz) {
#pragma unroll
        for (int c = 0; c < NC; ++c)
            if (c < ncols) Out[(size_t)c * ld + r] = -((a[c][0] + a[c][1]) + (a[c][2] + a[c][3]));
    }
}
inline void launch_neg_gm_batched(hipStream_t st, unsigned batch, int nz, int nzs, int ncols, const double* G, const double* M, double* Out,
                                  long sG, long sM) {
    const size_t lds = (size_t)ncols * nz * sizeof(double);
    if (nz <= 128 && ncols <= 4 && lds <= 48 * 1024) hipLaunchKernelGGL((k_neg_gm_cols<4>), dim3(1, batch), dim3(128), lds, st, nz, nzs, ncols, nzs, G, M, Out, sG, sM);
    else if (nz <= 128 && ncols <= 8 && lds <= 48 * 1024) hipLaunchKernelGGL((k_neg_gm_cols<8>), dim3(1, batch), dim3(128), lds, st, nz, nzs, ncols, nzs, G, M, Out, sG, sM);
    else if (nz <= 128 && ncols <= 16 && lds <= 48 * 1024) hipLaunchKernelGGL((k_neg_gm_cols<16>), dim3(1, batch), dim3(128), lds, st, nz, nzs, ncols, nzs, G, M, Out, sG, sM);
    else hipLaunchKernelGGL(k_neg_gm, dim3(4, batch), dim3(256), 0, st, nz, nzs, ncols, nzs, G, M, Out, sG, sM);
}

inline __global__ __launch_bounds__(256) void k_build_cprime(int mc, int nz, int nzs, int gs, const int* rowsel, const double* Gam,
                                                      const double* d, double* Cp) {
    for (int t = blockIdx.x * blockDim.x + threadIdx.x; t < mc * nzs; t += gridDim.x * blockDim.x) {
        const int r = t / nzs, c = t % nzs;
        Cp[t] = (c < nz) ? Gam[(size_t)rowsel[r] * gs + c] * d[c] : 0.0;
    }
}
inline __global__ __launch_bounds__(256) void k_cg(int mc, int nz, int nzs, const double* Cp, const double* G, double* CG) {
    for (int t = blockIdx.x * blockDim.x + threadIdx.x; t < mc * nzs; t += gridDim.x * blockDim.x) {
        const int r = t / nzs, c = t % nzs;
        double s = 0.0;
        if (c < nz)
            for (int j = 0; j < nz; ++j) s += Cp[(size_t)r * nzs + j] * G[(size_t)j * nzs + c];
        CG[t] = s;
    }
}
inline __global__ __launch_bounds__(256) void k_ghat(int nz, int mc, int nzs, int Rs, const double* G, const double* Cp,
                                              const double* CG, double* Ghat, double* gnorm) {
    const int R = nz + mc;
    for (int t = blockIdx.x * blockDim.x + threadIdx.x; t < R * Rs; t += gridDim.x * blockDim.x) {
        const int a = t / Rs, b = t % Rs;
        double v = 0.0;
        if (b < R) {
            if (a < nz && b < nz) v = G[(size_t)a * nzs + b];
            else if (a < nz) v = CG[(size_t)(b - nz) * nzs + a];
            else if (b < nz) v = CG[(size_t)(a - nz) * nzs + b];
            else
                for (int j = 0; j < nz; ++j) v += CG[(size_t)(a - nz) * nzs + j] * Cp[(size_t)(b - nz) * nzs + j];
        }
        Ghat[t] = v;
        if (a == b) gnorm[a] = sqrt(v > 0.0 ? v : 1.0);
    }
    for (int t = blockIdx.x * blockDim.x + threadIdx.x; t < Rs; t += gridDim.x * blockDim.x)
        if (t >= R) gnorm[t] = 1.0;
}

inline __global__ __launch_bounds__(256) void k_ghat_project(int R, int Rs, int ne, int eq0, const double* GhatE, const double* Y, double* Ghat,
                                                      double* gnorm) {
    for (int t = blockIdx.x * blockDim.x + threadIdx.x; t < R * Rs; t += gridDim.x * blockDim.x) {
        const int a = t / Rs, b = t % Rs;
        if (b >= R) continue;
        double v = Ghat[t];
        for (int e = 0; e < ne; ++e) v -= GhatE[(size_t)e * Rs + a] * Y[(size_t)e * Rs + b];
        if ((a >= eq0 && a < eq0 + ne) || (b >= eq0 && b < eq0 + ne)) v = 0.0;
        Ghat[t] = v;
        if (a == b) gnorm[a] = (a >= eq0 && a < eq0 + ne) ? 1.0 : sqrt(v > 0.0 ? v : 1.0);
    }
}

inline int design_shared_device(hipStream_t stream, int n, int m, int N, int nzs, int nrb, int ks, int ksf,
                                const std::vector<double>& A, const std::vector<double>& B, std::vector<double> Q,
                                std::vector<double> R, std::vector<double> S, std::vector<double> P, double rho,
                                double sigma, double* dMinvFrag, double* dVFrag, double* dHFrag, double* dFFrag,
                                double* dG, double* dD, std::vector<double>& hH, std::vector<double>& hF,
                                std::vector<double>& hd, std::string& err, const std::vector<int>& rowsel = std::vector<int>(),
                                int Rs = 0, double* dGhat = nullptr, double* dGnorm = nullptr, int rho_mode = 0,
                                double* dRho = nullptr, double* dVsOut = nullptr, double* dPlainOut = nullptr) {
    const int nz = m * N;
    const int useR = R[0] != 0.0, useS = useR && S[0] != 0.0;
    auto symmetrise = [](std::vector<double>& M, int k) {
        for (int j = 0; j < k; ++j)
            for (int i = 0; i < j; ++i) {
                const double v = 0.5 * (M[(size_t)j * k + i] + M[(size_t)i * k + j]);
                M[(size_t)j * k + i] = M[(size_t)i * k + j] = v;
            }
    };
    symmetrise(Q, n); symmetrise(P, n); symmetrise(R, m); symmetrise(S, m);
    const int njf = (n + 15) / 16, ps = 16 * njf, gs = nzs;
    const int kr = ((n * N + HESS_KC - 1) / HESS_KC) * HESS_KC;
    std::vector<void*> tmp;
    auto cleanup = [&]() { for (void* p : tmp) (void)hipFree(p); };
#define DTRY(call)                                                                           \
    do {                                                                                     \
        hipError_t e_ = (call);                                                              \
        if (e_ != hipSuccess) { err = std::string(#call) + ": " + hipGetErrorString(e_); cleanup(); return -3; } \
    } while (0)
    auto dnew = [&](double** p, size_t cnt) -> hipError_t {
        hipError_t e = hipMalloc(reinterpret_cast<void**>(p), cnt * sizeof(double) + 64);
        if (e == hipSuccess) { tmp.push_back(*p); e = hipMemsetAsync(*p, 0, cnt * sizeof(double), stream); }
        return e;
    };
    double *dA, *dB, *dQ, *dR, *dS, *dP, *dPhi, *dGk, *dGam, *dW, *dWP, *dH, *dF, *dHs, *dFs, *dVs, *dMinv;
    int* dFlag;
    DTRY(dnew(&dA, (size_t)n * n)); DTRY(dnew(&dB, (size_t)n * m)); DTRY(dnew(&dQ, (size_t)n * n));
    DTRY(dnew(&dR, (size_t)m * m)); DTRY(dnew(&dS, (size_t)m * m)); DTRY(dnew(&dP, (size_t)n * n));
    DTRY(dnew(&dPhi, (size_t)N * n * n)); DTRY(dnew(&dGk, (size_t)N * n * m));
    DTRY(dnew(&dGam, (size_t)kr * gs)); DTRY(dnew(&dW, (size_t)kr * gs)); DTRY(dnew(&dWP, (size_t)kr * ps));
    DTRY(dnew(&dH, (size_t)nz * nz)); DTRY(dnew(&dF, (size_t)nz * n));
    DTRY(dnew(&dHs, (size_t)nz * nzs)); DTRY(dnew(&dFs, (size_t)n * nzs)); DTRY(dnew(&dVs, (size_t)n * nzs)); DTRY(dnew(&dMinv, (size_t)nz * nzs));
    {
        double* f = nullptr;
        DTRY(dnew(&f, 8));
        dFlag = reinterpret_cast<int*>(f);
    }
    DTRY(hipMemcpyAsync(dA, A.data(), A.size() * sizeof(double), hipMemcpyHostToDevice, stream));
    DTRY(hipMemcpyAsync(dB, B.data(), B.size() * sizeof(double), hipMemcpyHostToDevice, stream));
    DTRY(hipMemcpyAsync(dQ, Q.data(), Q.size() * sizeof(double), hipMemcpyHostToDevice, stream));
    DTRY(hipMemcpyAsync(dR, R.data(), R.size() * sizeof(double), hipMemcpyHostToDevice, stream));
    DTRY(hipMemcpyAsync(dS, S.data(), S.size() * sizeof(double), hipMemcpyHostToDevice, stream));
    DTRY(hipMemcpyAsync(dP, P.data(), P.size() * sizeof(double), hipMemcpyHostToDevice, stream));

    hipLaunchKernelGGL(k_design_blocks, dim3(1), dim3(256), (size_t)(3 * n * n + n * m) * sizeof(double), stream, n, m, N,
                       dA, dB, dPhi, dGk, DesignStrides());
    DTRY(hipGetLastError());
    hipLaunchKernelGGL(k_design_gamma, dim3(N), dim3(256), 0, stream, n, m, N, dQ, dP, dPhi, dGk, dGam, dW, dWP, gs, ps, DesignStrides());
    DTRY(hipGetLastError());
    HessParams hp;
    hp.n = n; hp.m = m; hp.N = N; hp.nz = nz; hp.nrb = nrb; hp.njf = njf; hp.kr = kr;
    hp.Gam = dGam; hp.W = dW; hp.WP = dWP; hp.gs = gs; hp.ps = ps; hp.R = dR; hp.S = dS; hp.useR = useR; hp.useS = useS;
    hp.H = dH; hp.F = dF;
    const size_t hess_lds = (size_t)HESS_KC * (16 + (gs + 16) + (ps + 16)) * sizeof(double);
    hipLaunchKernelGGL(k_design_hessian, dim3(nrb), dim3(64 * (nrb + njf)), hess_lds, stream, hp);
    DTRY(hipGetLastError());
    hipLaunchKernelGGL(k_design_scale, dim3(1), dim3(256), 0, stream, nz, nzs, n, dH, dF, dD, dHs, dFs, dFlag, DesignStrides());
    DTRY(hipGetLastError());
    const size_t inv_lds = ((size_t)nz * (nz + 1) + nz + 2) * sizeof(double);
    DTRY(ensure_dyn_lds(reinterpret_cast<const void*>(k_design_inverse_chol), (size_t)(inv_lds)));
    hipLaunchKernelGGL(k_design_inverse_chol, dim3(1), dim3(512), inv_lds, stream, nz, nzs, dHs, 0.0, (const double*)nullptr, dG, dFlag, 0L, 0L, 0L, 0L);
    DTRY(hipGetLastError());
    hipLaunchKernelGGL(k_design_rho, dim3(1), dim3(256), 0, stream, nz, nzs, rho_mode, rho, dG, dRho, 0L, 0L);
    hipLaunchKernelGGL(k_design_inverse_chol, dim3(1), dim3(512), inv_lds, stream, nz, nzs, dHs, sigma, (const double*)dRho, dMinv, dFlag, 0L, 0L, 0L, 0L);
    DTRY(hipGetLastError());
    hipLaunchKernelGGL(k_pack_frags, dim3(32), dim3(256), 0, stream, dMinv, nz, nz, nzs, nrb, ks, dMinvFrag);
    hipLaunchKernelGGL(k_neg_gm, dim3(32), dim3(256), 0, stream, nz, nzs, n, nzs, dG, dFs, dVs, 0L, 0L);
    hipLaunchKernelGGL(k_pack_frags, dim3(32), dim3(256), 0, stream, dVs, nz, n, nzs, nrb, ksf, dVFrag);
    if (dVsOut) DTRY(hipMemcpyAsync(dVsOut, dVs, (size_t)n * nzs * sizeof(double), hipMemcpyDeviceToDevice, stream));
    if (dPlainOut) {
        const size_t mm = (size_t)nz * nzs, fv = (size_t)n * nzs;
        DTRY(hipMemcpyAsync(dPlainOut, dMinv, mm * sizeof(double), hipMemcpyDeviceToDevice, stream));
        DTRY(hipMemcpyAsync(dPlainOut + mm, dHs, mm * sizeof(double), hipMemcpyDeviceToDevice, stream));
        DTRY(hipMemcpyAsync(dPlainOut + 2 * mm, dFs, fv * sizeof(double), hipMemcpyDeviceToDevice, stream));
        DTRY(hipMemcpyAsync(dPlainOut + 2 * mm + fv, dVs, fv * sizeof(double), hipMemcpyDeviceToDevice, stream));
    }
    hipLaunchKernelGGL(k_pack_frags, dim3(32), dim3(256), 0, stream, dHs, nz, nz, nzs, nrb, ks, dHFrag);
    hipLaunchKernelGGL(k_pack_frags, dim3(32), dim3(256), 0, stream, dFs, nz, n, nzs, nrb, ksf, dFFrag);
    DTRY(hipGetLastError());
    if (!rowsel.empty()) {
        const int mc = (int)rowsel.size();
        double *dCp, *dCG;
        int* dSel;
        DTRY(dnew(&dCp, (size_t)mc * nzs)); DTRY(dnew(&dCG, (size_t)mc * nzs));
        {
            double* tmpi = nullptr;
            DTRY(dnew(&tmpi, (size_t)(mc + 1) / 2 + 1));
            dSel = reinterpret_cast<int*>(tmpi);
        }
        DTRY(hipMemcpyAsync(dSel, rowsel.data(), mc * sizeof(int), hipMemcpyHostToDevice, stream));
        hipLaunchKernelGGL(k_build_cprime, dim3(64), dim3(256), 0, stream, mc, nz, nzs, gs, dSel, dGam, dD, dCp);
        hipLaunchKernelGGL(k_cg, dim3(256), dim3(256), 0, stream, mc, nz, nzs, dCp, dG, dCG);
        hipLaunchKernelGGL(k_ghat, dim3(512), dim3(256), 0, stream, nz, mc, nzs, Rs, dG, dCp, dCG, dGhat, dGnorm);
        DTRY(hipGetLastError());
    }
    hH.assign((size_t)nz * nz, 0.0); hF.assign((size_t)nz * n, 0.0); hd.assign((size_t)nzs, 0.0);
    int flag = 0;
    DTRY(hipMemcpyAsync(hH.data(), dH, hH.size() * sizeof(double), hipMemcpyDeviceToHost, stream));
    DTRY(hipMemcpyAsync(hF.data(), dF, hF.size() * sizeof(double), hipMemcpyDeviceToHost, stream));
    DTRY(hipMemcpyAsync(hd.data(), dD, hd.size() * sizeof(double), hipMemcpyDeviceToHost, stream));
    DTRY(hipMemcpyAsync(&flag, dFlag, sizeof(int), hipMemcpyDeviceToHost, stream));
    DTRY(hipStreamSynchronize(stream));
#undef DTRY
    cleanup();
    if (flag != 0) {
        err = flag == 1 ? "design: condensed Hessian has a non-positive diagonal (R = 0 with an input that does not reach the cost?)"
                        : "design: Cholesky pivot not positive (Hessian not positive definite)";
        return -6;
    }
    return 0;
}

}
```

automationlabsmodelpredictivecontrol.jl_amd/csrc/almpc_kernels.hip.h:

```cpp
#pragma once
#include <hip/hip_runtime.h>
#include <stdint.h>

#include <map>
#include <mutex>
#include <utility>
#include <type_traits>

namespace almpc {

inline hipError_t ensure_dyn_lds(const void* fn, size_t bytes) {
    if (bytes <= 64 * 1024) return hipSuccess;
    static std::mutex mu;
    static std::map<std::pair<int, const void*>, size_t> cur;
    int dev = 0;
    hipError_t e = hipGetDevice(&dev);
    if (e != hipSuccess) return e;
    std::lock_guard<std::mutex> lock(mu);
    size_t& c = cur[std::make_pair(dev, fn)];
    if (c >= bytes) return hipSuccess;
    e = hipFuncSetAttribute(fn, hipFuncAttributeMaxDynamicSharedMemorySize, (int)bytes);
    if (e == hipSuccess) c = bytes;
    return e;
}


#ifdef ALMPC_STAMPS
__device__ long long* g_stamps = nullptr;
#define ALMPC_STAMP(WAVE_ID, SLOT)                                                                     \
    do {                                                                                               \
        __builtin_amdgcn_sched_barrier(0);                                                             \
        if (g_stamps && (threadIdx.x & 63) == 0) g_stamps[(size_t)(WAVE_ID) * 16 + (SLOT)] = __builtin_readcyclecounter(); \
        __builtin_amdgcn_sched_barrier(0);                                                             \
    } while (0)
#define ALMPC_ACC_DECL long long acc_t[8] = {0, 0, 0, 0, 0, 0, 0, 0}; long long acc_prev = 0; int acc_n = 0;
#define ALMPC_ACC_START do { __builtin_amdgcn_sched_barrier(0); acc_prev = __builtin_readcyclecounter(); __builtin_amdgcn_sched_barrier(0); } while (0)
#define ALMPC_ACC(SLOT) do { __builtin_amdgcn_sched_barrier(0); const long long n_ = __builtin_readcyclecounter(); acc_t[SLOT] += n_ - acc_prev; acc_prev = n_; __builtin_amdgcn_sched_barrier(0); } while (0)
#define ALMPC_ACC_FLUSH(WAVE_ID) do { if (g_stamps && (threadIdx.x & 63) == 0) { for (int i_ = 0; i_ < 8; ++i_) g_stamps[(size_t)(4096 + (WAVE_ID)) * 16 + i_] = acc_t[i_]; g_stamps[(size_t)(4096 + (WAVE_ID)) * 16 + 8] = acc_n; } } while (0)
#else
#define ALMPC_STAMP(WAVE_ID, SLOT) do { } while (0)
#define ALMPC_ACC_DECL
#define ALMPC_ACC_START do { } while (0)
#define ALMPC_ACC(SLOT) do { } while (0)
#define ALMPC_ACC_FLUSH(WAVE_ID) do { } while (0)
#endif

__host__ __device__ inline int packed_tri_off(int nz, int c) {
    const int full = c * nz - (c * (c - 1)) / 2;
    const int pads = (nz & 1) ? (c / 2) : ((c + 1) / 2);
    return full + pads;
}
__host__ __device__ inline long packed_tri_doubles(int nz) { return ((long)packed_tri_off(nz, nz) + 1) & ~1L; }

typedef double d4 __attribute__((ext_vector_type(4)));
typedef double d2v __attribute__((ext_vector_type(2)));

constexpr int TILE = 16;

__device__ __forceinline__ d4 mfma_f64(double a, double b, d4 c) {
    return __builtin_amdgcn_mfma_f64_16x16x4f64(a, b, c, 0, 0, 0);
}

template <int KS>
__device__ __forceinline__ d4 tile_matmul(const double (&a)[KS], const double* bbuf, int q, int col) {
    d4 acc0 = {0.0, 0.0, 0.0, 0.0}, acc1 = {0.0, 0.0, 0.0, 0.0};
#pragma unroll
    for (int ks = 0; ks < KS; ks += 2) {
        double b0 = bbuf[(4 * ks + q) * TILE + col];
        acc0 = mfma_f64(a[ks], b0, acc0);
        if (ks + 1 < KS) {
            double b1 = bbuf[(4 * (ks + 1) + q) * TILE + col];
            acc1 = mfma_f64(a[ks + 1], b1, acc1);
        }
    }
    return acc0 + acc1;
}

__device__ __forceinline__ double qmax(double v) {
    v = fmax(v, __shfl_xor(v, 16));
    v = fmax(v, __shfl_xor(v, 32));
    return v;
}

struct AdmmParams {
    int nz, n, m, batch, nzs;
    const double* MinvFrag;
    const double* VFrag;
    const double* v0S;
    long v0S_stride;
    const double* HFrag;
    const double* FFrag;
    int ksf;
    const double* dvec;
    const double* rhovec;
    const double* umin;
    const double* umax;
    const double* uref;
    long uref_stride;
    const double* xref;
    long xref_stride;
    const double* fS;
    long fS_stride;
    const double* x0;
    double* xs;
    double* zs;
    double* ys;
    double* v0;
    int32_t* status;
    int32_t* iters;
    int32_t* piters;
    int32_t* perm;
    double rho, sigma, alpha, eps_abs, eps_rel;
    int max_iter, check_every, warm;
    int keep_state;
    uint32_t* yflags;
};

template <int NRB, int KS, typename AfterRequests>
__device__ __forceinline__ void admm_body(const AdmmParams& p, double* smem, AfterRequests after_requests) {
    constexpr int RP = 16 * NRB;
    static_assert(4 * KS <= RP, "K padding must fit the row padding");
    double* rhs0 = smem;
    double* rhs1 = smem + RP * TILE;
    double* red = smem + 2 * RP * TILE;
    double* e0s = red + NRB * 8 * TILE;

    const int wv = threadIdx.x >> 6, lane = threadIdx.x & 63;
    const int col = lane & 15, q = lane >> 4;
    const int inst = blockIdx.x * TILE + col;
    const bool valid = inst < p.batch;
    const int instc = valid ? inst : p.batch - 1;
    ALMPC_STAMP(blockIdx.x * NRB + wv, 0);

    constexpr int KSF_MAX = 16;
    double af[KSF_MAX];
#pragma unroll
    for (int ks = 0; ks < KSF_MAX; ++ks)
        af[ks] = (ks < p.ksf) ? p.FFrag[((size_t)(wv * p.ksf + ks)) * 64 + lane] : 0.0;
    int row[4];
    double dv[4], dinv[4], lo[4], hi[4], fs[4], rho[4];
#pragma unroll
    for (int i = 0; i < 4; ++i) {
        row[i] = wv * 16 + q + 4 * i;
        const bool in = row[i] < p.nz;
        const int r = in ? row[i] : 0;
        dv[i] = in ? p.dvec[r] : 1.0;
        rho[i] = p.rhovec[r];
        const double ur = p.uref[(size_t)instc * p.uref_stride + r];
        lo[i] = p.umin[r % p.m] - ur;
        hi[i] = p.umax[r % p.m] - ur;
        fs[i] = in ? p.fS[(size_t)instc * p.fS_stride + r] : 0.0;
    }
    const int kpf = 4 * p.ksf;
    for (int t = threadIdx.x; t < kpf * TILE; t += blockDim.x) {
        int k = t / TILE, c = t % TILE;
        int ii = blockIdx.x * TILE + c;
        if (ii >= p.batch) ii = p.batch - 1;
        double v = 0.0;
        if (k < p.n) v = p.x0[(size_t)ii * p.n + k] - p.xref[(size_t)ii * p.xref_stride + k];
        e0s[t] = v;
    }
    double a[KS];
#pragma unroll
    for (int ks = 0; ks < KS; ++ks) a[ks] = p.MinvFrag[((size_t)(wv * KS + ks)) * 64 + lane];
    after_requests();
    ALMPC_STAMP(blockIdx.x * NRB + wv, 5);
    __syncthreads();
    ALMPC_STAMP(blockIdx.x * NRB + wv, 6);

    {
        d4 acc = {0.0, 0.0, 0.0, 0.0};
#pragma unroll
        for (int ks = 0; ks < KSF_MAX; ++ks)
            if (ks < p.ksf) acc = mfma_f64(af[ks], e0s[(4 * ks + q) * TILE + col], acc);
#pragma unroll
        for (int i = 0; i < 4; ++i) {
            const bool in = row[i] < p.nz;
            dinv[i] = 1.0 / dv[i];
            lo[i] = in ? lo[i] * dinv[i] : 0.0;
            hi[i] = in ? hi[i] * dinv[i] : 0.0;
            fs[i] = in ? acc[i] + fs[i] : 0.0;
        }
    }

    ALMPC_STAMP(blockIdx.x * NRB + wv, 7);
    double x[4], z[4], yt[4], px[4], rown[4];
    const double sigma = p.sigma, alpha = p.alpha;
    if (p.warm) {
#pragma unroll
        for (int i = 0; i < 4; ++i) {
            const size_t o = (size_t)instc * p.nzs + row[i];
            x[i] = p.xs[o];
            yt[i] = p.ys[o];
            z[i] = p.zs[o];
        }
#pragma unroll
        for (int i = 0; i < 4; ++i) {
            yt[i] = yt[i] / rho[i];
            z[i] = fmin(fmax(z[i], lo[i]), hi[i]);
            rhs0[row[i] * TILE + col] = x[i];
        }
        __syncthreads();
        d4 acc = {0.0, 0.0, 0.0, 0.0};
#pragma unroll
        for (int ks0 = 0; ks0 < KS; ks0 += 8) {
            double ah[8];
#pragma unroll
            for (int u = 0; u < 8; ++u)
                if (ks0 + u < KS) ah[u] = p.HFrag[((size_t)(wv * KS + ks0 + u)) * 64 + lane];
#pragma unroll
            for (int u = 0; u < 8; ++u)
                if (ks0 + u < KS) acc = mfma_f64(ah[u], rhs0[(4 * (ks0 + u) + q) * TILE + col], acc);
        }
#pragma unroll
        for (int i = 0; i < 4; ++i) px[i] = acc[i];
        __syncthreads();
    } else {
#pragma unroll
        for (int i = 0; i < 4; ++i) x[i] = z[i] = yt[i] = px[i] = 0.0;
    }
#pragma unroll
    for (int i = 0; i < 4; ++i) {
        rown[i] = sigma * x[i] - fs[i] + rho[i] * (z[i] - yt[i]);
        rhs0[row[i] * TILE + col] = rown[i];
    }
    {
        double mf = 0.0;
#pragma unroll
        for (int i = 0; i < 4; ++i) mf = fmax(mf, fabs(fs[i] * dinv[i]));
        mf = qmax(mf);
        if (q == 0) red[(wv * 8 + 7) * TILE + col] = mf;
    }
    __syncthreads();
    double nf = 0.0;
    for (int w2 = 0; w2 < NRB; ++w2) nf = fmax(nf, red[(w2 * 8 + 7) * TILE + col]);
    __syncthreads();

    ALMPC_STAMP(blockIdx.x * NRB + wv, 1);
    bool active = true;
    int my_iters = p.max_iter, my_status = 1;
    double* cur = rhs0;
    double* nxt = rhs1;
    for (int it = 1; it <= p.max_iter; ++it) {
        const d4 xt4 = tile_matmul<KS>(a, cur, q, col);
#pragma unroll
        for (int i = 0; i < 4; ++i) {
            const double xt = xt4[i];
            if (active) {
                const double hxt = rown[i] - (sigma + rho[i]) * xt;
                px[i] = alpha * hxt + (1.0 - alpha) * px[i];
                x[i] = alpha * xt + (1.0 - alpha) * x[i];
                const double w = alpha * xt + (1.0 - alpha) * z[i] + yt[i];
                const double zn = fmin(fmax(w, lo[i]), hi[i]);
                yt[i] = w - zn;
                z[i] = zn;
                rown[i] = sigma * x[i] - fs[i] + rho[i] * (z[i] - yt[i]);
            }
            nxt[row[i] * TILE + col] = rown[i];
        }
        const bool check = (it % p.check_every == 0) || (it == p.max_iter);
        if (check) {
            double m_rp = 0, m_x = 0, m_z = 0, m_rd = 0, m_hx = 0, m_y = 0, m_bad = 0;
#pragma unroll
            for (int i = 0; i < 4; ++i) {
                m_rp = fmax(m_rp, fabs(dv[i] * (x[i] - z[i])));
                m_x = fmax(m_x, fabs(dv[i] * x[i]));
                m_z = fmax(m_z, fabs(dv[i] * z[i]));
                const double yi = rho[i] * yt[i];
                m_rd = fmax(m_rd, fabs((px[i] + fs[i] + yi) * dinv[i]));
                m_hx = fmax(m_hx, fabs(px[i] * dinv[i]));
                m_y = fmax(m_y, fabs(yi * dinv[i]));
                const double s = x[i] + yi + px[i];
                if (!(fabs(s) <= 1.79e308)) m_bad = 1.0;
            }
            m_rp = qmax(m_rp); m_x = qmax(m_x); m_z = qmax(m_z); m_rd = qmax(m_rd);
            m_hx = qmax(m_hx); m_y = qmax(m_y); m_bad = qmax(m_bad);
            if (q == 0) {
                double* r = red + wv * 8 * TILE + col;
                r[0 * TILE] = m_rp; r[1 * TILE] = m_x; r[2 * TILE] = m_z; r[3 * TILE] = m_rd;
                r[4 * TILE] = m_hx; r[5 * TILE] = m_y; r[6 * TILE] = m_bad;
            }
        }
        __syncthreads();
        if (check) {
            double rp = 0, nx = 0, nzn = 0, rd = 0, nhx = 0, ny = 0, bad = 0;
            for (int w2 = 0; w2 < NRB; ++w2) {
                const double* r = red + w2 * 8 * TILE + col;
                rp = fmax(rp, r[0 * TILE]); nx = fmax(nx, r[1 * TILE]); nzn = fmax(nzn, r[2 * TILE]);
                rd = fmax(rd, r[3 * TILE]); nhx = fmax(nhx, r[4 * TILE]); ny = fmax(ny, r[5 * TILE]);
                bad = fmax(bad, r[6 * TILE]);
            }
            if (active) {
                const bool conv = (rp <= p.eps_abs + p.eps_rel * fmax(nx, nzn)) &&
                                  (rd <= p.eps_abs + p.eps_rel * fmax(fmax(nhx, ny), nf));
                if (bad > 0.0) { active = false; my_iters = it; my_status = 2; }
                else if (conv) { active = false; my_iters = it; my_status = 0; }
            }
            const bool any_active = __any(active);
            __syncthreads();
            if (!any_active) { double* t = cur; cur = nxt; nxt = t; break; }
        }
        double* t = cur; cur = nxt; nxt = t;
    }

    ALMPC_STAMP(blockIdx.x * NRB + wv, 2);
#pragma unroll
    for (int ks = 0; ks < KSF_MAX; ++ks)
        af[ks] = (ks < p.ksf) ? p.VFrag[((size_t)(wv * p.ksf + ks)) * 64 + lane] : 0.0;
    double v0s[4];
#pragma unroll
    for (int i = 0; i < 4; ++i) v0s[i] = (row[i] < p.nz) ? p.v0S[(size_t)instc * p.v0S_stride + row[i]] : 0.0;
    if (valid && wv == 0 && q == 0) {
        p.iters[inst] = my_iters;
        p.status[inst] = my_status;
        p.piters[inst] = 0;
    }
    {
        int cntf = 0;
#pragma unroll
        for (int i = 0; i < 4; ++i) cntf += (row[i] < p.nz && yt[i] != 0.0) ? 1 : 0;
        cntf += __shfl_xor(cntf, 16);
        cntf += __shfl_xor(cntf, 32);
        if (q == 0) red[(wv * 8 + 0) * TILE + col] = (double)cntf;
    }
    __syncthreads();
    if (wv == 0 && q == 0) {
        int k0 = valid ? 0 : -1;
        if (valid)
            for (int w2 = 0; w2 < NRB; ++w2) k0 += (int)red[(w2 * 8 + 0) * TILE + col];
        red[(0 * 8 + 1) * TILE + col] = (double)k0;
        __builtin_amdgcn_fence(__ATOMIC_RELEASE, "wavefront");
        __builtin_amdgcn_wave_barrier();
        __builtin_amdgcn_fence(__ATOMIC_ACQUIRE, "wavefront");
        int rank = 0;
        for (int c2 = 0; c2 < TILE; ++c2) {
            const int ko = (int)red[(0 * 8 + 1) * TILE + c2];
            rank += (ko > k0 || (ko == k0 && c2 < col)) ? 1 : 0;
        }
        p.perm[blockIdx.x * TILE + rank] = valid ? inst : -1;
    }
    d4 v04 = {v0s[0], v0s[1], v0s[2], v0s[3]};
#pragma unroll
    for (int ks = 0; ks < KSF_MAX; ++ks)
        if (ks < p.ksf) v04 = mfma_f64(af[ks], e0s[(4 * ks + q) * TILE + col], v04);
    ALMPC_STAMP(blockIdx.x * NRB + wv, 3);

    constexpr int TS = RP + 2;
    static_assert(TILE * TS <= 2 * RP * TILE, "staging tile must fit the two rhs buffers");
    double* stage = smem;
    auto flush = [&](const double (&v)[4], double* dst) {
        __syncthreads();
#pragma unroll
        for (int i = 0; i < 4; ++i) stage[col * TS + row[i]] = v[i];
        __syncthreads();
        for (int e = 2 * threadIdx.x; e < TILE * RP; e += 2 * blockDim.x) {
            const int ci = e / RP, r = e % RP;
            const int ii = blockIdx.x * TILE + ci;
            if (ii < p.batch)
                *reinterpret_cast<d2v*>(dst + (size_t)ii * p.nzs + r) = *reinterpret_cast<const d2v*>(stage + ci * TS + r);
        }
    };
    const double v0r[4] = {v04[0], v04[1], v04[2], v04[3]};
    double y[4];
#pragma unroll
    for (int i = 0; i < 4; ++i) y[i] = rho[i] * yt[i];
    if (p.keep_state) {
        flush(x, p.xs);
        flush(y, p.ys);
    } else {
        uint32_t mk = 0;
#pragma unroll
        for (int i = 0; i < 4; ++i) {
            const uint32_t b = (uint32_t)(q + 4 * i);
            mk |= (yt[i] < 0.0 ? 1u : 0u) << b;
            mk |= (yt[i] > 0.0 ? 1u : 0u) << (16u + b);
        }
        mk |= (uint32_t)__shfl_xor((int)mk, 16);
        mk |= (uint32_t)__shfl_xor((int)mk, 32);
        if (q == 0 && valid) p.yflags[(size_t)inst * NRB + wv] = mk;
    }
    flush(z, p.zs);
    flush(v0r, p.v0);
    ALMPC_STAMP(blockIdx.x * NRB + wv, 4);
}

template <int NRB, int KS>
__global__ __launch_bounds__(64 * NRB) void k_admm(AdmmParams p) {
    extern __shared__ __attribute__((aligned(16))) double smem[];
    admm_body<NRB, KS>(p, smem, []() {});
}

struct RolloutParams {
    int n, m, N, batch, nzs;
    const double* A;
    const double* B;
    long A_stride = 0, B_stride = 0, d_stride = 0;
    const double* dvec;
    const double* w;
    const double* x0;
    const double* xref;
    long xref_stride;
    const double* uref;
    long uref_stride;
    const double* umin;
    const double* umax;
    double* x;
    double* ex;
    double* u;
    double* eu;
};

struct PolishParams {
    int nz, m, batch, nzs;
    const double* G;
    const double* dvec;
    const double* umin;
    const double* umax;
    const double* uref;
    long uref_stride;
    const double* zs;
    const double* ys;
    const uint32_t* yflags;
    int yflag_words;
    const double* v0;
    double* w;
    int32_t* status;
    int32_t* piters;
// ... 777 lines not shown
#pragma unroll
        for (int t = 0; t < 16; ++t) {
            Sg[(16 * hhf + t) * 64 + hpos] = Sr[t];
            Sg[(16 * hhf + t) * 64 + 32 + hpos] = 0.0;
        }
#pragma unroll 4
        for (int c = 32; c < cap2; ++c) Sg[c * 64 + lane] = 0.0;
        if (lane >= 32 && lane < cap2) Sg[lane * 64 + lane] = 1.0;
        if (lane >= 32) lam = 0.0;
        sync_s(PolishMode<true>{});
    };

    const int s0 = (in0 && y0 < 0.0 && w0 <= lo0) ? -1 : ((in0 && y0 > 0.0 && w0 >= hi0) ? 1 : 0);
    const int s1 = (in1 && y1 < 0.0 && w1 <= lo1) ? -1 : ((in1 && y1 > 0.0 && w1 >= hi1) ? 1 : 0);
    const unsigned long long m0 = __ballot(s0 != 0), m1 = __ballot(s1 != 0);
    const int k0 = __popcll(m0) + __popcll(m1);
    bool give_up = skip || k0 > 64;
    if (!give_up && k0 > 0) {
        using M = PolishMode<false>;
        const M m{};
        const int pos = lane & 31;
        const unsigned long long below = (lane == 0) ? 0ull : (~0ull >> (64 - lane));
        const int p0 = __popcll(m0 & below) + __popcll(m1 & below), p1 = p0 + (s0 != 0 ? 1 : 0);
        int* ibuf = reinterpret_cast<int*>(rowbuf);
        if (s0 != 0) { ibuf[p0] = r0; ibuf[64 + p0] = s0; }
        if (s1 != 0) { ibuf[p1] = r1; ibuf[64 + p1] = s1; }
        wave_fence_lds();
        bool started = false;
        if constexpr (START) {
            if (p.start_rows && k0 > 32) {
                const int32_t* sr = GL(p.start_rows) + (size_t)inst * 65;
                const bool same = sr[0] == k0 && (lane >= k0 || sr[1 + lane] == ibuf[lane]);
                if (__all(same)) {
                    started = true;
                    k = k0;
                    wrow = lane < k0 ? ibuf[lane] : 0;
                    wsd = lane < k0 ? ibuf[64 + lane] : 0;
                    wave_fence_lds();
                    if (s0 != 0) { act0 = true; bnd0 = s0 > 0 ? hi0 : lo0; }
                    if (s1 != 0) { act1 = true; bnd1 = s1 > 0 ? hi1 : lo1; }
                    put_rows(s0 > 0 ? hi0 : lo0, s1 > 0 ? hi1 : lo1);
                    wbnd = lane < k0 ? rowbuf[wrow] : 0.0;
                    lam = 0.0;
                    wrow_s[lane] = wrow;
                    const double* src = GL(p.sglobal) + (size_t)inst * POLISH_GLB_PER_INST;
                    if (Sg != src) {
                        for (int c = 0; c < 64; c += 8) {
                            double v[8];
#pragma unroll
                            for (int t = 0; t < 8; ++t) v[t] = src[(c + t) * 64 + lane];
#pragma unroll
                            for (int t = 0; t < 8; ++t) Sg[(c + t) * 64 + lane] = v[t];
                        }
                    }
                    sync_s(PolishMode<true>{});
                    recompute(PolishMode<true>{});
                    overflow = true;
                }
            }
        }
        if (!started) {
        k = k0 < 32 ? k0 : 32;
        if (pos < k) { wrow = ibuf[pos]; wsd = ibuf[64 + pos]; }
        const int pend_row = (lane >= 32 && lane < k0) ? ibuf[lane] : 0;
        const int pend_sd = (lane >= 32 && lane < k0) ? ibuf[64 + lane] : 0;
        wave_fence_lds();
        if (s0 != 0 && p0 < 32) { act0 = true; bnd0 = s0 > 0 ? hi0 : lo0; }
        if (s1 != 0 && p1 < 32) { act1 = true; bnd1 = s1 > 0 ? hi1 : lo1; }
        put_rows(s0 > 0 ? hi0 : lo0, s1 > 0 ? hi1 : lo1);
        if (pos < k) wbnd = rowbuf[wrow];
        const double pend_bnd = (lane >= 32 && lane < k0) ? rowbuf[pend_row] : 0.0;
        for (int pass = 0; pass < 2; ++pass) {
        if (lane < 32) wrow_s[lane] = (lane < k) ? wrow : 0;
        {
            double gv[16];
#pragma unroll
            for (int t = 0; t < 16; ++t) gv[t] = Gp[wrow_s[16 * hhf + t] * gs + wrow];
#pragma unroll
            for (int t = 0; t < 16; ++t) Sr[t] = (16 * hhf + t < k && pos < k) ? gv[t] : 0.0;
        }
#pragma unroll 1
        for (int hh = 0; hh < 2; ++hh) {
#pragma unroll
            for (int tj = 0; tj < 16; ++tj) {
                const int pv = 16 * hh + tj;
                if (pv < k) {
                    if (hhf == hh) {
                        pbufa[hpos] = Sr[tj];
                        pbufb[hpos] = (hpos < pv) ? -Sr[tj] : Sr[tj];
                    }
                    wave_fence_lds();
                    const double fcol = pbufa[hpos], piv = pbufa[pv];
                    double rowpv[16];
                    bcast16(pbufb, rowpv);
                    const double ip = fast_rcp_d(piv);
                    const bool isp = hpos == pv;
                    const double f = isp ? 0.0 : fcol * ip;
                    const double scale = isp ? ip : 1.0;
#pragma unroll
                    for (int t = 0; t < 16; ++t) Sr[t] = __builtin_fma(-f, rowpv[t], Sr[t]) * scale;
                    Sr[tj] = (hhf == hh) ? (isp ? ip : -f) : Sr[tj];
                }
            }
        }
        recompute(m);
        if (pass == 1 || k0 > 32) break;
        {
            const bool mine = lane < 32 && pos < k;
            const double viol = mine ? ((wsd > 0) ? -lam : lam) : -__builtin_inf();
            const double lmax = wave_max(mine ? fabs(lam) : 0.0);
            const bool bad = mine && viol > 1e-12 * fmax(1.0, lmax);
            const unsigned badm = (unsigned)__ballot(bad);
            const int nb = __popc(badm);
            if (nb < 2) break;
            const unsigned usedm = (k >= 32) ? 0xffffffffu : ((1u << k) - 1u);
            const unsigned keepm = usedm & ~badm;
            put_rows(0.0, 0.0);
            if (bad) rowbuf[wrow] = 1.0;
            wave_fence_lds();
            {
                const d2 mk = *reinterpret_cast<const d2*>(rowbuf + r0);
                if (mk[0] != 0.0) act0 = false;
                if (mk[1] != 0.0) act1 = false;
            }
            const bool keep = lane < 32 && ((keepm >> pos) & 1u) != 0u;
            const int np = __popc(keepm & ((1u << pos) - 1u));
            if (keep) { ibuf[np] = wrow; ibuf[64 + np] = wsd; pbufa[np] = wbnd; }
            wave_fence_lds();
            k = __popc(keepm);
            wrow = 0; wsd = 0; wbnd = 0.0; lam = 0.0;
            if (pos < k) { wrow = ibuf[pos]; wsd = ibuf[64 + pos]; wbnd = pbufa[pos]; }
            wave_fence_lds();
            it += nb;
        }
        }
        if (k0 > 32) {
            tier2_home(k0);
            to_global();
            for (int q = 32; q < k0; ++q)
                add_row(PolishMode<true>{}, __builtin_amdgcn_readlane(pend_row, q), readlane_d(pend_bnd, q),
                        __builtin_amdgcn_readlane(pend_sd, q));
            fresh = false;
            overflow = true;
        }
        }
    }
    ALMPC_STAMP(inst, 10);
    if (!give_up) {
        if (!overflow) {
            run(PolishMode<false>{});
            if (overflow) { tier2_home(33); to_global(); }
        }
        if (overflow) {
            overflow = false;
            run(PolishMode<true>{});
            if (overflow && own_slot) {
                slot_to_global();
                overflow = false;
                run(PolishMode<true>{});
            }
            give_up = overflow;
        }
    }
    if constexpr (GLDS) {
        if (own_slot) {
            if (lane == 0) atomicExch(qcnt + 1, -1);
            own_slot = false;
        }
    }
// ... 331 lines not shown
```

Before: 16850 batch-steps/s (one step = 4096 instance QP solves).

## Precompute first ADMM iterate via Minv*V and pair pivots in polish sweep

Adds a design-time product of the dense inverse with the V matrix (W1) and its per-reference shift, so on cold start the first ADMM iteration's tile matmul is replaced by an MFMA against the same right-hand side used for the initial projection. The v0 computation is also moved up and fused into that same MFMA loop, with the first few fragments kept in registers. Separately, the polish Gauss-Jordan sweep now eliminates two pivots per LDS round trip, which halves the number of fences. This costs extra registers and a second device buffer, and the peeled path only applies when the reference is shared (not batched).

Result: no change. 16970 batch-steps/s (one step = 4096 instance QP solves), median of 6 (+0.7%).

```diff
diff --git a/automationlabsmodelpredictivecontrol.jl_amd/csrc/almpc_api.hip b/automationlabsmodelpredictivecontrol.jl_amd/csrc/almpc_api.hip
--- a/automationlabsmodelpredictivecontrol.jl_amd/csrc/almpc_api.hip
+++ b/automationlabsmodelpredictivecontrol.jl_amd/csrc/almpc_api.hip
@@ -47,6 +47,9 @@
     double rho = 0.1, sigma = 1e-6;
     std::vector<double> H, F, P, d;
     double *dMinvFrag = nullptr, *dVFrag = nullptr, *dHFrag = nullptr, *dFFrag = nullptr, *dG = nullptr;
+    double *dW1Frag = nullptr, *dMinvDense = nullptr, *dW1S = nullptr;
+    size_t w1s_cap = 0;
+    bool w1_ok = false;
     double *dD = nullptr, *dUmin = nullptr, *dUmax = nullptr, *dA = nullptr, *dB = nullptr;
     double *dXref = nullptr, *dUref = nullptr, *dFS = nullptr, *dV0S = nullptr, *dRho = nullptr;
     size_t ref_cap[3] = {0, 0, 0};
@@ -265,7 +268,7 @@
 
 void free_all(almpc_handle* h) {
     io_free(h);
-    void* ptrs[] = {h->dMinvFrag, h->dVFrag, h->dHFrag, h->dFFrag, h->dG, h->dD, h->dUmin, h->dUmax, h->dA, h->dB,
+    void* ptrs[] = {h->dW1Frag, h->dMinvDense, h->dW1S, h->dMinvFrag, h->dVFrag, h->dHFrag, h->dFFrag, h->dG, h->dD, h->dUmin, h->dUmax, h->dA, h->dB,
                     h->dXref, h->dUref, h->dFS, h->dV0S, h->dRho, h->dRollM, h->dX0, h->dXs, h->dZs, h->dYs, h->dV0, h->dW, h->dX, h->dEx,
                     h->dU, h->dEu, h->dStatus, h->dIters, h->dPiters, h->dPerm, h->dYflags, h->dSglobal, h->dStartRows, h->dGhat, h->dGnorm, h->dXmin,
                     h->dXmax, h->dRowTraj, h->dRowEq, h->dRowXidx, h->dRowState, h->dRowMap, h->dGhatE, h->dWinvE, h->lA, h->lB, h->lC, h->lE, h->bA, h->bB, h->bMinv, h->bG, h->bHs, h->bFs,
@@ -1019,6 +1022,7 @@
         return ALMPC_OK;
     }
     TRY(dalloc(&h->dMinvFrag, fr)); TRY(dalloc(&h->dVFrag, (size_t)h->nrb * h->ksf * 64)); TRY(dalloc(&h->dHFrag, fr));
+    TRY(dalloc(&h->dW1Frag, (size_t)h->nrb * h->ksf * 64)); TRY(dalloc(&h->dMinvDense, (size_t)h->nz * h->nzs));
     TRY(dalloc(&h->dFFrag, (size_t)h->nrb * h->ksf * 64));
     TRY(dalloc(&h->dG, (size_t)h->nz * h->nzs));
     TRY(dalloc(&h->dD, (size_t)h->nzs)); TRY(dalloc(&h->dRho, (size_t)h->nzs)); TRY(dalloc(&h->dUmin, (size_t)m)); TRY(dalloc(&h->dUmax, (size_t)m));
@@ -1167,6 +1171,7 @@
     if ((xmin == nullptr) != (xmax == nullptr)) return fail(h, ALMPC_ERR_INVALID, "design: give both xmin and xmax or neither");
     if (!(rho > 0.0) || !(sigma >= 0.0)) return fail(h, ALMPC_ERR_INVALID, "design: rho must be > 0 and sigma >= 0");
     h->designed = false;
+    h->w1_ok = false;
     h->sqp.ready = h->sqp.started = false;
     h->relin.ready = false;
     HIP_TRY(h, hipSetDevice(h->device));
@@ -1197,7 +1202,7 @@
     if (!rowsel.empty() && !h->dVsPlain) HIP_TRY(h, dalloc(&h->dVsPlain, (size_t)n * h->nzs));
     if (h->nzs <= 64 && !h->dPlain) HIP_TRY(h, dalloc(&h->dPlain, 2 * (size_t)h->nz * h->nzs + 2 * (size_t)n * h->nzs));
     int rc = design_shared_device(h->stream, n, m, N, h->nzs, h->nrb, h->ks, h->ksf, Am, Bm, Qm, Rm, Sm, Pm, rho, sigma,
-                                  h->dMinvFrag, h->dVFrag, h->dHFrag, h->dFFrag, h->dG, h->dD, h->H, h->F, h->d, h->err,
+                                  h->dMinvFrag, h->dVFrag, h->dW1Frag, h->dMinvDense, h->dHFrag, h->dFFrag, h->dG, h->dD, h->H, h->F, h->d, h->err,
                                   rowsel, h->Rs, h->dGhat, h->dGnorm, h->rho_mode, h->dRho, rowsel.empty() ? nullptr : h->dVsPlain,
                                   h->nzs <= 64 ? h->dPlain : nullptr);
     if (rc != ALMPC_OK) return rc;
@@ -1765,7 +1770,7 @@
     h->designed = false;
     hipLaunchKernelGGL(k_fs_scale, dim3(256), dim3(256), 0, h->stream, h->batch, nz, nzs, h->bQ, (long)nz, h->bD, h->dFS);
     hipLaunchKernelGGL(k_neg_gm, dim3(1, (unsigned)h->batch), dim3(256), 0, h->stream, nz, nzs, 1, nz, h->bG, h->dFS, h->dV0S,
-                       (long)nz * nzs, (long)nz);
+                       (long)nz * nzs, (long)nz, (const double*)nullptr, (double*)nullptr);
     HIP_TRY(h, hipGetLastError());
     HIP_TRY(h, hipStreamSynchronize(h->stream));
     h->ltv = true;
@@ -1928,7 +1933,10 @@
 AdmmParams admm_params(const almpc_handle* h, const almpc_opts& o, bool keep_state) {
     AdmmParams ap;
     ap.nz = h->nz; ap.n = h->n; ap.m = h->m; ap.batch = h->batch; ap.nzs = h->nzs;
-    ap.MinvFrag = h->dMinvFrag; ap.VFrag = h->dVFrag; ap.v0S = h->dV0S; ap.v0S_stride = h->fS_stride; ap.HFrag = h->dHFrag; ap.FFrag = h->dFFrag; ap.ksf = h->ksf;
+    ap.MinvFrag = h->dMinvFrag; ap.VFrag = h->dVFrag; ap.v0S = h->dV0S; ap.v0S_stride = h->fS_stride;
+    const bool w1 = h->w1_ok && !h->batched;
+    ap.W1Frag = w1 ? h->dW1Frag : nullptr; ap.w1S = w1 ? h->dW1S : nullptr; ap.w1S_stride = h->fS_stride;
+    ap.HFrag = h->dHFrag; ap.FFrag = h->dFFrag; ap.ksf = h->ksf;
     ap.dvec = h->dD; ap.rhovec = h->dRho; ap.umin = h->dUmin; ap.umax = h->dUmax;
     ap.uref = h->dUref; ap.uref_stride = h->uref_stride; ap.xref = h->dXref; ap.xref_stride = h->xref_stride;
     ap.fS = h->dFS; ap.fS_stride = h->fS_stride; ap.x0 = h->dX0;
@@ -2566,7 +2574,7 @@
     if (q.useS) {
         hipLaunchKernelGGL(k_fs_scale, dim3(256), dim3(256), 0, st, h->batch, nz, nzs, q.gS, 0L, h->bD, h->dFS);
         hipLaunchKernelGGL(k_neg_gm, dim3(1, (unsigned)h->batch), dim3(256), 0, st, nz, nzs, 1, nz, h->bG, h->dFS, h->dV0S,
-                           (long)nz * nzs, (long)nz);
+                           (long)nz * nzs, (long)nz, (const double*)nullptr, (double*)nullptr);
         HIP_TRY(h, hipGetLastError());
     }
     if (timing) HIP_TRY(h, hipEventRecord(q.ev[2], st));
@@ -3081,7 +3089,7 @@
         launch_batched_factor(h, ds, h->rho, h->sigma, st, mode.guess != Guess::Admm, ltv_scales, false, v0_in_inverse ? h->dFS : nullptr, h->dV0S);
         if (h->mc > 0) HIP_TRY(h, launch_ghat_inst(h, q.A, q.B));
         if (!ltv_scales) hipLaunchKernelGGL(k_fs_scale, dim3(256), dim3(256), 0, st, h->batch, nz, nzs, h->bQ, (long)nz, h->bD, h->dFS);
-        if (!v0_in_inverse) hipLaunchKernelGGL(k_neg_gm, dim3(1, (unsigned)b), dim3(256), 0, st, nz, nzs, 1, nz, h->bG, h->dFS, h->dV0S, (long)nz * nzs, (long)nz);
+        if (!v0_in_inverse) hipLaunchKernelGGL(k_neg_gm, dim3(1, (unsigned)b), dim3(256), 0, st, nz, nzs, 1, nz, h->bG, h->dFS, h->dV0S, (long)nz * nzs, (long)nz, (const double*)nullptr, (double*)nullptr);
         HIP_TRY(h, hipGetLastError());
         h->designed = true;
         const int rc = calculate_checked(h, opts, mode);
@@ -3209,6 +3217,7 @@
     h->sqp.ready = h->sqp.started = false;
     h->relin.ready = false;
     h->designed = false;
+    h->w1_ok = false;
     const size_t fcnt = h->batched ? (size_t)h->batch : cnt;
     if (!(h->dXref && h->dUref && h->dFS && h->dV0S && h->ref_cap[0] == cnt * xs && h->ref_cap[1] == cnt * us && h->ref_cap[2] == fcnt * us)) {
         if (h->dXref) { (void)hipFree(h->dXref); h->dXref = nullptr; }
@@ -3252,7 +3261,7 @@
             hipLaunchKernelGGL(k_fs_scale, dim3(256), dim3(256), 0, h->stream, h->batch, nz, h->nzs, dGs, per_instance ? (long)us : 0L,
                                h->bD, h->dFS);
             hipLaunchKernelGGL(k_neg_gm, dim3(1, (unsigned)h->batch), dim3(256), 0, h->stream, nz, h->nzs, 1, (int)us, h->bG, h->dFS,
-                               h->dV0S, (long)nz * h->nzs, (long)us);
+                               h->dV0S, (long)nz * h->nzs, (long)us, (const double*)nullptr, (double*)nullptr);
             e = hipGetLastError();
             if (e == hipSuccess) e = hipStreamSynchronize(h->stream);
         }
@@ -3260,13 +3269,20 @@
         if (e != hipSuccess) return fail(h, ALMPC_ERR_HIP, std::string("set_reference (batched): ") + hipGetErrorString(e));
     } else {
     HIP_TRY(h, hipMemcpy(h->dFS, fS.data(), cnt * us * sizeof(double), hipMemcpyHostToDevice));
+    if (h->w1s_cap != cnt * us) {
+        if (h->dW1S) { (void)hipFree(h->dW1S); h->dW1S = nullptr; }
+        h->w1s_cap = 0;
+        HIP_TRY(h, dalloc(&h->dW1S, cnt * us));
+        h->w1s_cap = cnt * us;
+    }
     {
         const size_t blocks = (cnt * us + 255) / 256;
         hipLaunchKernelGGL(k_neg_gm, dim3((unsigned)(blocks < 1024 ? blocks : 1024)), dim3(256), 0, h->stream, nz, h->nzs,
-                           (int)cnt, (int)us, h->dG, h->dFS, h->dV0S, 0L, 0L);
+                           (int)cnt, (int)us, h->dG, h->dFS, h->dV0S, 0L, 0L, (const double*)h->dMinvDense, h->dW1S);
         HIP_TRY(h, hipGetLastError());
         HIP_TRY(h, hipStreamSynchronize(h->stream));
     }
+    h->w1_ok = true;
     }
     h->xref_stride = per_instance ? (long)xs : 0;
     h->uref_stride = per_instance ? (long)us : 0;
diff --git a/automationlabsmodelpredictivecontrol.jl_amd/csrc/almpc_design.hip.h b/automationlabsmodelpredictivecontrol.jl_amd/csrc/almpc_design.hip.h
--- a/automationlabsmodelpredictivecontrol.jl_amd/csrc/almpc_design.hip.h
+++ b/automationlabsmodelpredictivecontrol.jl_amd/csrc/almpc_design.hip.h
@@ -761,19 +761,27 @@
 }
 
 inline __global__ __launch_bounds__(256) void k_pack_frags(const double* M, int rows, int cols, int ld, int nrb, int ks,
-                                                    double* frag) {
+                                                    double* frag, const double* M2, double* frag2) {
     const int total = nrb * ks * 64;
-    for (int t = blockIdx.x * blockDim.x + threadIdx.x; t < total; t += gridDim.x * blockDim.x) {
+    for (int t2 = blockIdx.x * blockDim.x + threadIdx.x; t2 < (M2 ? 2 * total : total); t2 += gridDim.x * blockDim.x) {
+        const bool second = t2 >= total;
+        const int t = second ? t2 - total : t2;
         const int l = t & 63, s = (t >> 6) % ks, rb = (t >> 6) / ks;
         const int r = rb * 16 + (l & 15), c = 4 * s + (l >> 4);
-        frag[t] = (r < rows && c < cols) ? M[(size_t)c * ld + r] : 0.0;
-    }
-}
-
-inline __global__ __launch_bounds__(256) void k_neg_gm(int nz, int nzs, int ncols, int ld, const double* G, const double* M, double* Out,
-                                                long sG, long sM) {
-    G += blockIdx.y * sG; M += blockIdx.y * sM; Out += blockIdx.y * sM;
-    for (long t = (long)blockIdx.x * blockDim.x + threadIdx.x; t < (long)ncols * nz; t += (long)gridDim.x * blockDim.x) {
+        const double* src = second ? M2 : M;
+        (second ? frag2 : frag)[t] = (r < rows && c < cols) ? src[(size_t)c * ld + r] : 0.0;
+    }
+}
+
+inline __global__ __launch_bounds__(256) void k_neg_gm(int nz, int nzs, int ncols, int ld, const double* G_, const double* M, double* Out_,
+                                                long sG, long sM, const double* G2, double* Out2) {
+    const long total = (long)ncols * nz;
+    M += blockIdx.y * sM;
+    for (long t2 = (long)blockIdx.x * blockDim.x + threadIdx.x; t2 < (G2 ? 2 * total : total); t2 += (long)gridDim.x * blockDim.x) {
+        const bool second = t2 >= total;
+        const long t = second ? t2 - total : t2;
+        const double* G = (second ? G2 : G_) + blockIdx.y * sG;
+        double* Out = (second ? Out2 : Out_) + blockIdx.y * sM;
         const int c = (int)(t / nz), r = (int)(t % nz);
         const double* mcol = M + (size_t)c * ld;
         double a0 = 0.0, a1 = 0.0, a2 = 0.0, a3 = 0.0;
@@ -836,7 +844,7 @@
     if (nz <= 128 && ncols <= 4 && lds <= 48 * 1024) hipLaunchKernelGGL((k_neg_gm_cols<4>), dim3(1, batch), dim3(128), lds, st, nz, nzs, ncols, nzs, G, M, Out, sG, sM);
     else if (nz <= 128 && ncols <= 8 && lds <= 48 * 1024) hipLaunchKernelGGL((k_neg_gm_cols<8>), dim3(1, batch), dim3(128), lds, st, nz, nzs, ncols, nzs, G, M, Out, sG, sM);
     else if (nz <= 128 && ncols <= 16 && lds <= 48 * 1024) hipLaunchKernelGGL((k_neg_gm_cols<16>), dim3(1, batch), dim3(128), lds, st, nz, nzs, ncols, nzs, G, M, Out, sG, sM);
-    else hipLaunchKernelGGL(k_neg_gm, dim3(4, batch), dim3(256), 0, st, nz, nzs, ncols, nzs, G, M, Out, sG, sM);
+    else hipLaunchKernelGGL(k_neg_gm, dim3(4, batch), dim3(256), 0, st, nz, nzs, ncols, nzs, G, M, Out, sG, sM, (const double*)nullptr, (double*)nullptr);
 }
 
 inline __global__ __launch_bounds__(256) void k_build_cprime(int mc, int nz, int nzs, int gs, const int* rowsel, const double* Gam,
@@ -891,8 +899,8 @@
 inline int design_shared_device(hipStream_t stream, int n, int m, int N, int nzs, int nrb, int ks, int ksf,
                                 const std::vector<double>& A, const std::vector<double>& B, std::vector<double> Q,
                                 std::vector<double> R, std::vector<double> S, std::vector<double> P, double rho,
-                                double sigma, double* dMinvFrag, double* dVFrag, double* dHFrag, double* dFFrag,
-                                double* dG, double* dD, std::vector<double>& hH, std::vector<double>& hF,
+                                double sigma, double* dMinvFrag, double* dVFrag, double* dW1Frag, double* dMinv, double* dHFrag,
+                                double* dFFrag, double* dG, double* dD, std::vector<double>& hH, std::vector<double>& hF,
                                 std::vector<double>& hd, std::string& err, const std::vector<int>& rowsel = std::vector<int>(),
                                 int Rs = 0, double* dGhat = nullptr, double* dGnorm = nullptr, int rho_mode = 0,
                                 double* dRho = nullptr, double* dVsOut = nullptr, double* dPlainOut = nullptr) {
@@ -920,14 +928,15 @@
         if (e == hipSuccess) { tmp.push_back(*p); e = hipMemsetAsync(*p, 0, cnt * sizeof(double), stream); }
         return e;
     };
-    double *dA, *dB, *dQ, *dR, *dS, *dP, *dPhi, *dGk, *dGam, *dW, *dWP, *dH, *dF, *dHs, *dFs, *dVs, *dMinv;
+    double *dA, *dB, *dQ, *dR, *dS, *dP, *dPhi, *dGk, *dGam, *dW, *dWP, *dH, *dF, *dHs, *dFs, *dVs, *dW1s;
     int* dFlag;
     DTRY(dnew(&dA, (size_t)n * n)); DTRY(dnew(&dB, (size_t)n * m)); DTRY(dnew(&dQ, (size_t)n * n));
     DTRY(dnew(&dR, (size_t)m * m)); DTRY(dnew(&dS, (size_t)m * m)); DTRY(dnew(&dP, (size_t)n * n));
     DTRY(dnew(&dPhi, (size_t)N * n * n)); DTRY(dnew(&dGk, (size_t)N * n * m));
     DTRY(dnew(&dGam, (size_t)kr * gs)); DTRY(dnew(&dW, (size_t)kr * gs)); DTRY(dnew(&dWP, (size_t)kr * ps));
     DTRY(dnew(&dH, (size_t)nz * nz)); DTRY(dnew(&dF, (size_t)nz * n));
-    DTRY(dnew(&dHs, (size_t)nz * nzs)); DTRY(dnew(&dFs, (size_t)n * nzs)); DTRY(dnew(&dVs, (size_t)n * nzs)); DTRY(dnew(&dMinv, (size_t)nz * nzs));
+    DTRY(dnew(&dHs, (size_t)nz * nzs)); DTRY(dnew(&dFs, (size_t)n * nzs)); DTRY(dnew(&dVs, (size_t)n * nzs)); DTRY(dnew(&dW1s, (size_t)n * nzs));
+    DTRY(hipMemsetAsync(dMinv, 0, (size_t)nz * nzs * sizeof(double), stream));
     {
         double* f = nullptr;
         DTRY(dnew(&f, 8));
@@ -961,9 +970,9 @@
     hipLaunchKernelGGL(k_design_rho, dim3(1), dim3(256), 0, stream, nz, nzs, rho_mode, rho, dG, dRho, 0L, 0L);
     hipLaunchKernelGGL(k_design_inverse_chol, dim3(1), dim3(512), inv_lds, stream, nz, nzs, dHs, sigma, (const double*)dRho, dMinv, dFlag, 0L, 0L, 0L, 0L);
     DTRY(hipGetLastError());
-    hipLaunchKernelGGL(k_pack_frags, dim3(32), dim3(256), 0, stream, dMinv, nz, nz, nzs, nrb, ks, dMinvFrag);
-    hipLaunchKernelGGL(k_neg_gm, dim3(32), dim3(256), 0, stream, nz, nzs, n, nzs, dG, dFs, dVs, 0L, 0L);
-    hipLaunchKernelGGL(k_pack_frags, dim3(32), dim3(256), 0, stream, dVs, nz, n, nzs, nrb, ksf, dVFrag);
+    hipLaunchKernelGGL(k_pack_frags, dim3(32), dim3(256), 0, stream, dMinv, nz, nz, nzs, nrb, ks, dMinvFrag, (const double*)nullptr, (double*)nullptr);
+    hipLaunchKernelGGL(k_neg_gm, dim3(32), dim3(256), 0, stream, nz, nzs, n, nzs, dG, dFs, dVs, 0L, 0L, (const double*)dMinv, dW1s);
+    hipLaunchKernelGGL(k_pack_frags, dim3(32), dim3(256), 0, stream, dVs, nz, n, nzs, nrb, ksf, dVFrag, (const double*)dW1s, dW1Frag);
     if (dVsOut) DTRY(hipMemcpyAsync(dVsOut, dVs, (size_t)n * nzs * sizeof(double), hipMemcpyDeviceToDevice, stream));
     if (dPlainOut) {
         const size_t mm = (size_t)nz * nzs, fv = (size_t)n * nzs;
@@ -972,8 +981,8 @@
         DTRY(hipMemcpyAsync(dPlainOut + 2 * mm, dFs, fv * sizeof(double), hipMemcpyDeviceToDevice, stream));
         DTRY(hipMemcpyAsync(dPlainOut + 2 * mm + fv, dVs, fv * sizeof(double), hipMemcpyDeviceToDevice, stream));
     }
-    hipLaunchKernelGGL(k_pack_frags, dim3(32), dim3(256), 0, stream, dHs, nz, nz, nzs, nrb, ks, dHFrag);
-    hipLaunchKernelGGL(k_pack_frags, dim3(32), dim3(256), 0, stream, dFs, nz, n, nzs, nrb, ksf, dFFrag);
+    hipLaunchKernelGGL(k_pack_frags, dim3(32), dim3(256), 0, stream, dHs, nz, nz, nzs, nrb, ks, dHFrag, (const double*)nullptr, (double*)nullptr);
+    hipLaunchKernelGGL(k_pack_frags, dim3(32), dim3(256), 0, stream, dFs, nz, n, nzs, nrb, ksf, dFFrag, (const double*)nullptr, (double*)nullptr);
     DTRY(hipGetLastError());
     if (!rowsel.empty()) {
         const int mc = (int)rowsel.size();
diff --git a/automationlabsmodelpredictivecontrol.jl_amd/csrc/almpc_kernels.hip.h b/automationlabsmodelpredictivecontrol.jl_amd/csrc/almpc_kernels.hip.h
--- a/automationlabsmodelpredictivecontrol.jl_amd/csrc/almpc_kernels.hip.h
+++ b/automationlabsmodelpredictivecontrol.jl_amd/csrc/almpc_kernels.hip.h
@@ -88,6 +88,9 @@
     const double* VFrag;
     const double* v0S;
     long v0S_stride;
+    const double* W1Frag;
+    const double* w1S;
+    long w1S_stride;
     const double* HFrag;
     const double* FFrag;
     int ksf;
@@ -133,12 +136,19 @@
     ALMPC_STAMP(blockIdx.x * NRB + wv, 0);
 
     constexpr int KSF_MAX = 16;
-    double af[KSF_MAX];
+    const bool peel = !p.warm && p.W1Frag != nullptr;
+    constexpr int KSF_HOIST = 4;
+    double af[KSF_MAX], avf[KSF_HOIST], awf[KSF_HOIST];
 #pragma unroll
     for (int ks = 0; ks < KSF_MAX; ++ks)
         af[ks] = (ks < p.ksf) ? p.FFrag[((size_t)(wv * p.ksf + ks)) * 64 + lane] : 0.0;
+#pragma unroll
+    for (int ks = 0; ks < KSF_HOIST; ++ks) {
+        avf[ks] = (ks < p.ksf) ? p.VFrag[((size_t)(wv * p.ksf + ks)) * 64 + lane] : 0.0;
+        awf[ks] = (peel && ks < p.ksf) ? p.W1Frag[((size_t)(wv * p.ksf + ks)) * 64 + lane] : 0.0;
+    }
     int row[4];
-    double dv[4], dinv[4], lo[4], hi[4], fs[4], rho[4];
+    double dv[4], dinv[4], lo[4], hi[4], fs[4], rho[4], v0s[4], w1s[4];
 #pragma unroll
     for (int i = 0; i < 4; ++i) {
         row[i] = wv * 16 + q + 4 * i;
@@ -150,6 +160,8 @@
         lo[i] = p.umin[r % p.m] - ur;
         hi[i] = p.umax[r % p.m] - ur;
         fs[i] = in ? p.fS[(size_t)instc * p.fS_stride + r] : 0.0;
+        v0s[i] = in ? p.v0S[(size_t)instc * p.v0S_stride + r] : 0.0;
+        w1s[i] = (peel && in) ? p.w1S[(size_t)instc * p.w1S_stride + r] : 0.0;
     }
     const int kpf = 4 * p.ksf;
     for (int t = threadIdx.x; t < kpf * TILE; t += blockDim.x) {
@@ -168,11 +180,23 @@
     __syncthreads();
     ALMPC_STAMP(blockIdx.x * NRB + wv, 6);
 
+    d4 v04 = {v0s[0], v0s[1], v0s[2], v0s[3]};
+    d4 xt1 = {w1s[0], w1s[1], w1s[2], w1s[3]};
     {
         d4 acc = {0.0, 0.0, 0.0, 0.0};
 #pragma unroll
         for (int ks = 0; ks < KSF_MAX; ++ks)
-            if (ks < p.ksf) acc = mfma_f64(af[ks], e0s[(4 * ks + q) * TILE + col], acc);
+            if (ks < p.ksf) {
+                const double b = e0s[(4 * ks + q) * TILE + col];
+                acc = mfma_f64(af[ks], b, acc);
+                if (ks < KSF_HOIST) {
+                    v04 = mfma_f64(avf[ks], b, v04);
+                    if (peel) xt1 = mfma_f64(awf[ks], b, xt1);
+                } else {
+                    v04 = mfma_f64(p.VFrag[((size_t)(wv * p.ksf + ks)) * 64 + lane], b, v04);
+                    if (peel) xt1 = mfma_f64(p.W1Frag[((size_t)(wv * p.ksf + ks)) * 64 + lane], b, xt1);
+                }
+            }
 #pragma unroll
         for (int i = 0; i < 4; ++i) {
             const bool in = row[i] < p.nz;
@@ -242,7 +266,7 @@
     double* cur = rhs0;
     double* nxt = rhs1;
     for (int it = 1; it <= p.max_iter; ++it) {
-        const d4 xt4 = tile_matmul<KS>(a, cur, q, col);
+        const d4 xt4 = (peel && it == 1) ? xt1 : tile_matmul<KS>(a, cur, q, col);
 #pragma unroll
         for (int i = 0; i < 4; ++i) {
             const double xt = xt4[i];
@@ -301,15 +325,10 @@
             if (!any_active) { double* t = cur; cur = nxt; nxt = t; break; }
         }
         double* t = cur; cur = nxt; nxt = t;
+        if (it == 1) ALMPC_STAMP(blockIdx.x * NRB + wv, 15);
     }
 
     ALMPC_STAMP(blockIdx.x * NRB + wv, 2);
-#pragma unroll
-    for (int ks = 0; ks < KSF_MAX; ++ks)
-        af[ks] = (ks < p.ksf) ? p.VFrag[((size_t)(wv * p.ksf + ks)) * 64 + lane] : 0.0;
-    double v0s[4];
-#pragma unroll
-    for (int i = 0; i < 4; ++i) v0s[i] = (row[i] < p.nz) ? p.v0S[(size_t)instc * p.v0S_stride + row[i]] : 0.0;
     if (valid && wv == 0 && q == 0) {
         p.iters[inst] = my_iters;
         p.status[inst] = my_status;
@@ -339,10 +358,6 @@
         }
         p.perm[blockIdx.x * TILE + rank] = valid ? inst : -1;
     }
-    d4 v04 = {v0s[0], v0s[1], v0s[2], v0s[3]};
-#pragma unroll
-    for (int ks = 0; ks < KSF_MAX; ++ks)
-        if (ks < p.ksf) v04 = mfma_f64(af[ks], e0s[(4 * ks + q) * TILE + col], v04);
     ALMPC_STAMP(blockIdx.x * NRB + wv, 3);
 
     constexpr int TS = RP + 2;
@@ -1286,9 +1301,38 @@
 #pragma unroll 1
         for (int hh = 0; hh < 2; ++hh) {
 #pragma unroll
-            for (int tj = 0; tj < 16; ++tj) {
+            for (int tj = 0; tj < 16; tj += 2) {
                 const int pv = 16 * hh + tj;
-                if (pv < k) {
+                if (pv + 1 < k) {
+                    const bool own = hhf == hh, isp = hpos == pv, isq = hpos == pv + 1;
+                    const double ip = fast_rcp_d(readlane_d(Sr[tj], 32 * hh + pv));
+                    const double aqp = readlane_d(Sr[tj], 32 * hh + pv + 1);
+                    const double sc1 = isp ? ip : 1.0;
+                    if (own) {
+                        const double ca = Sr[tj];
+                        const double cq = __builtin_fma(-(isp ? 0.0 : ca * ip), aqp, Sr[tj + 1]) * sc1;
+                        pbufa[hpos] = ca;
+                        pbufa[32 + hpos] = cq;
+                        pbufb[hpos] = (hpos < pv) ? -ca : ca;
+                        pbufb[32 + hpos] = (hpos <= pv) ? -cq : cq;
+                    }
+                    wave_fence_lds();
+                    const double f1 = isp ? 0.0 : pbufa[hpos] * ip;
+                    const double iq = fast_rcp_d(pbufa[32 + pv + 1]);
+                    const double f2 = isq ? 0.0 : pbufa[32 + hpos] * iq;
+                    const double sc2 = isq ? iq : 1.0;
+                    double rp[16], rq[16];
+                    bcast16(pbufb, rp);
+                    bcast16(pbufb + 32, rq);
+#pragma unroll
+                    for (int t = 0; t < 16; ++t) {
+                        double v = __builtin_fma(-f1, rp[t], Sr[t]) * sc1;
+                        if (t == tj) v = own ? (isp ? ip : -f1) : v;
+                        v = __builtin_fma(-f2, rq[t], v) * sc2;
+                        if (t == tj + 1) v = own ? (isq ? iq : -f2) : v;
+                        Sr[t] = v;
+                    }
+                } else if (pv < k) {
                     if (hhf == hh) {
                         pbufa[hpos] = Sr[tj];
                         pbufb[hpos] = (hpos < pv) ? -Sr[tj] : Sr[tj];
```
